# amathislab/HOISDF

Hardware: AMD Instinct MI355X
Metric: samples/sec (img + 2048 SDF queries) fwd+bwd at 1/2/4/8 MI355X (higher is better)
Workload: dtype f32 (emulated contractions, f32 accumulate, f16x2 form: operands as scaled hi + lo f16 pieces x 3 products - 22 operand bits, one power-of-two scale per ROW of a linear layer's row operand, per (sample, head) of the attention operands, per weight matrix; the attention backward's dS as three pieces x

## Files before the change

hoisdf_amd/_lib.py:

```python
from __future__ import annotations

import ctypes as C
import os
from typing import Dict, List

_HERE = os.path.dirname(os.path.abspath(__file__))
LIB_PATH = os.environ.get("HOISDF_LIB", os.path.join(_HERE, "libhoisdf_hip.so"))
HEADER_PATH = os.path.join(os.path.dirname(_HERE), "include", "hoisdf.h")
MAX_LEVELS = 8


class HoisdfLibraryError(RuntimeError):
    pass


class HoisdfError(RuntimeError):
    def __init__(self, code: int, msg: str):
        super().__init__(f"libhoisdf_hip status {code}: {msg}")
        self.code = code


class Pyramid(C.Structure):
    _fields_ = [("n_levels", C.c_int), ("B", C.c_int), ("data", C.c_void_p * MAX_LEVELS),
                ("C", C.c_int * MAX_LEVELS), ("H", C.c_int * MAX_LEVELS), ("W", C.c_int * MAX_LEVELS)]
# ... 157 lines not shown
    "hoisdf_attention_bwd": [_P, _I, _P, _I, _P, _I, _P, _I, _P, _I, _P, _P, _P, _P, _P, _I, _I, _I, _I,
                             _I, _F, _U64, _P],
    "hoisdf_attention_fwd_bf16x2": [_P, _I, _P, _I, _P, _I, _P, _I, _I, _I, _I, _I, _I, _P, _L, _P],
    "hoisdf_attention_fwd_emu": [_P, _I, _P, _I, _P, _I, _P, _I, _P, _I, _I, _I, _I, _I, _F, _U64, _P, _L, _I, _P],
    "hoisdf_attention_fwd_emu_mag": [_P, _I, _P, _I, _P, _I, _P, _I, _P, _I, _I, _I, _I, _I, _F, _U64, _P, _L, _I, _P, _P, _P, _P, _P],
    "hoisdf_attention_bwd_emu": [_P, _I, _P, _I, _P, _I, _P, _I, _P, _I, _P, _P, _P, _P, _P, _I, _I, _I, _I, _I, _F, _U64, _P, _P,
                                 _L, _P],
    "hoisdf_attention_bwd_emu_mag": [_P, _I, _P, _I, _P, _I, _P, _I, _P, _I, _P, _P, _P, _P, _P, _I, _I, _I, _I, _I, _F, _U64, _P, _P,
                                 _L, _P, _P, _P, _P, _P, _P],
    "hoisdf_attention_small_fwd": [_P, _I, _P, _I, _P, _I, _P, _P, _I, _P, _I, _I, _I, _I, _F, _U64, _P],
    "hoisdf_attention_small_bwd": [_P, _I, _P, _I, _P, _I, _P, _P, _I, _P, _P, _P, _I, _I, _I, _I, _F,
                                   _U64, _P],
    "hoisdf_add_layernorm_fwd": [_P, _P, _P, _P, _P, _P, _P, _L, _I, _F, _F, _U64, _P],
    "hoisdf_add_layernorm_bwd": [_P, _P, _P, _P, _P, _P, _P, _P, _P, _P, _P, _L, _I, _F, _U64, _P],
    "hoisdf_residual_dropout": [_P, _P, _P, _L, _I, _F, _U64, _P],
    "hoisdf_layernorm_rows_fwd": [_P, _P, _P, _P, _P, _P, _L, _I, _I, _I, _F, _P],
    "hoisdf_layernorm_rows_bwd": [_P, _P, _P, _P, _P, _P, _P, _P, _P, _L, _I, _I, _I, _P],
    "hoisdf_sdf_query_train_fwd": [_PYR, _P, _P, _L, _I, _P, _P, _F, _I, _I, _SDFW, _F, _F, _U64, _P, _P, _P, _P, _L, _P, _L, _P],
    "hoisdf_sdf_query_bwd": [_PYR, _P, _P, _L, _I, _P, _P, _F, _I, _I, _SDFW, _F, _F, _P, _L, _P, _P, _P, _L, _P],
    "hoisdf_sdf_infer_count": [_P, _P, _P, _F, _I, _I, _P, _P, _P, _P],
    "hoisdf_sdf_infer_count_begin": [_P, _P, _P, _F, _I, _I, _P, _P, _P],
    "hoisdf_sdf_infer": [_PYR, _P, _P, _P, _F, _I, _I, _P, _P, _I, _I, _I, _SDFW, _F, _F, _U64, _P, _P, _P, _P, _L, _P],
    "hoisdf_decoder_layer_fwd": [_P, _P, _P, _P, _P, _P, _P, _P, _P, _L, _P, _L, _P],
    "hoisdf_decoder_layer_bwd": [_P, _P, _P, _P, _P, _P, _P, _L, _P, _P, _P, _P, _I, _P, _P, _P, _L, _P],
    "hoisdf_encoder_layer_fwd": [_P, _P, _P, _P, _P, _P, _L, _P, _L, _P],
    "hoisdf_encoder_layer_bwd": [_P, _P, _P, _P, _P, _L, _P, _P, _P, _P, _P, _L, _P],
    "hoisdf_mano_prepare": [_P, _P, _P, _P, _P],
    "hoisdf_mano_head_fwd": [_P, _I, _I, _P, _I, _I, _P, _P, _P, _P, _P, _P, _P, _P, _P, _I, _I, _P, _P, _P, _P, _P],
    "hoisdf_mano_head_bwd": [_P, _P, _I, _P, _P, _P, _P, _P, _P, _P, _P, _P, _I, _I, _P, _P, _P, _P, _P, _P, _P],
    "hoisdf_vote_fwd": [_P, _P, _P, _P, _P, _I, _I, _I, _I, _P],
    "hoisdf_vote_bwd": [_P, _P, _P, _P, _P, _P, _P, _P, _I, _I, _I, _I, _P],
    "hoisdf_vote_loss_fwd": [_P, _P, _P, _P, _F, _P, _P, _P, _P, _P, _I, _I, _I, _I, _P],
    "hoisdf_vote_loss_bwd": [_P, _P, _P, _P, _F, _P, _P, _P, _P, _P, _P, _P, _I, _I, _I, _I, _P],
    "hoisdf_tokens_fwd": [_P, _P, _P, _P, _F, _I, _I, _P, _P, _P, _P, _P, _P, _P, _P, _P, _I, _I, _I, _I, _I, _P, _L, _P, _L, _P],
    "hoisdf_tokens_bwd": [_P, _P, _P, _P, _F, _I, _I, _P, _P, _P, _P, _P, _P, _L, _P, _P, _I, _P, _I, _I, _I, _I, _I, _P, _L, _P],
    "hoisdf_heads_vote_fwd": [_P, _P, _P, _P, _P, _F, _P, _P, _P, _P, _I, _I, _I, _I, _P, _L, _P, _L, _P],
    "hoisdf_heads_vote_bwd": [_P, _P, _P, _P, _P, _F, _P, _P, _L, _P, _P, _P, _P, _P, _P, _I, _I, _I, _I, _P, _L, _P],
    "hoisdf_point_loss_fwd": [_P, _P, _L, _L, _I, _L, _I, _F, _F, _F, _P, _P, _P],
    "hoisdf_point_loss_bwd": [_P, _P, _L, _L, _I, _L, _I, _F, _F, _F, _P, _P, _P],
    "hoisdf_pose_prepare": [_P, _P, _P, _L, _P],
    "hoisdf_pose_infer_begin": [_P, _P, _P, _P, _P, _P, _P, _P, _P],
    "hoisdf_pose_infer": [_P, _P, _PYR, _P, _P, _P, _P, _P, _P, _P, _P, _P, _L, _P, _P],
    "hoisdf_conv_pack_weight": [_P, _P, _P, _P, _P, _P, _F, _I, _I, _I, _I, _I, _P, _P, _P],
    "hoisdf_conv_plan": [_L, _I, _I, _I, _P, _P],
    "hoisdf_conv2d_fwd": [_P, _I, _P, _P, _P, _I, _P, _I, _I, _I, _I, _I, _I, _I, _I, _I, _I, _I, _I, _P, _L, _P],
    "hoisdf_conv_transpose2d_fwd": [_P, _I, _P, _P, _P, _I, _I, _I, _I, _I, _I, _I, _I, _P, _L, _P],
    "hoisdf_maxpool2d_fwd": [_P, _I, _P, _I, _I, _I, _I, _I, _P],
    "hoisdf_encoder_prepare": [_P, _P, _I, _P, _L, _P],
    "hoisdf_encoder_pyramid_shape": [_P, _PYR],
    "hoisdf_encoder_infer": [_P, _P, _P, _P, _P, _P, _L, _P],
}
_RET = {"hoisdf_version": C.c_char_p, "hoisdf_last_error": C.c_char_p}
_OTHER = {"hoisdf_set_deterministic": ([_I], None), "hoisdf_set_gemm_emu": ([_I], None), "hoisdf_get_gemm_emu": ([], C.c_int), "hoisdf_get_deterministic": ([], C.c_int),
          "hoisdf_mano_dirs_image_floats": ([], C.c_long),
          "hoisdf_point_loss_blocks": ([_L], C.c_int),
          "hoisdf_bn_workspace_floats": ([_L, _I], C.c_long),
          "hoisdf_token_build_bwd_partials": ([], C.c_int),
          "hoisdf_tokens_saved_bytes": ([_P, _L, _I], C.c_long),
          "hoisdf_tokens_workspace_bytes": ([_P, _L, _I], C.c_long),
          "hoisdf_heads_vote_saved_bytes": ([_P, _P, _I, _I, _I, _I], C.c_long),
          "hoisdf_heads_vote_workspace_bytes": ([_P, _P, _I, _I, _I, _I, _I], C.c_long),
          "hoisdf_sdf_infer_workspace": ([_L, _I, _I], C.c_long),
          "hoisdf_sdf_query_train_saved_bytes": ([_L, _I], C.c_long),
          "hoisdf_sdf_query_train_workspace_bytes": ([_L, _I, _I], C.c_long),
          "hoisdf_decoder_layer_saved_bytes": ([_P], C.c_long),
          "hoisdf_decoder_layer_workspace_bytes": ([_P, _I], C.c_long),
          "hoisdf_encoder_layer_saved_bytes": ([_P], C.c_long),
          "hoisdf_encoder_layer_out_mag": ([_P, _P], C.c_void_p),
          "hoisdf_encoder_layer_workspace_bytes": ([_P, _I], C.c_long),
          "hoisdf_sdf_query_workspace": ([_L, _I, _I], C.c_long),
          "hoisdf_linear_bwd_weight_workspace": ([_L, _I, _I], C.c_long),
          "hoisdf_linear_emu_image_bytes": ([_I, _I], C.c_long),
          "hoisdf_linear_emu_prepare_blocks": ([_I, _I, _I], C.c_long),
          "hoisdf_linear_bwd_weight_emu_workspace": ([_L, _I, _I], C.c_long),
          "hoisdf_linear_emu_supported": ([_P, _L, _I], C.c_int),
          "hoisdf_linear_emu_small_max_rows": ([], C.c_int),
          "hoisdf_linear_emu_pieces": ([], C.c_int),
          "hoisdf_mag_words": ([_L], C.c_long),
          "hoisdf_head_mag_words": ([_L, _I, _I], C.c_long),
          "hoisdf_linear_emu_small_supported": ([_P, _L, _P, _L, _L, _I, _I], C.c_int),
          "hoisdf_attention_bf16x2_workspace": ([_I, _I, _I, _I], C.c_long),
          "hoisdf_attention_emu_workspace": ([_I, _I, _I, _I, _I], C.c_long),
          "hoisdf_attention_bwd_emu_workspace": ([_I, _I, _I, _I, _I], C.c_long),
          "hoisdf_conv_packed_floats": ([_I, _I, _I, _I], C.c_long),
          "hoisdf_conv_workspace_bytes": ([_L, _I, _I, _I], C.c_long),
          "hoisdf_encoder_tensor_count": ([_P], C.c_int),
          "hoisdf_encoder_tensor_name": ([_P, _I], C.c_char_p),
          "hoisdf_encoder_tensor_numel": ([_P, _I], C.c_long),
          "hoisdf_encoder_prepared_bytes": ([_P], C.c_long),
          "hoisdf_encoder_infer_workspace": ([_P], C.c_long),
          "hoisdf_encoder_launch_count": ([_P], C.c_int),
          "hoisdf_pose_prepared_bytes": ([_P], C.c_long),
          "hoisdf_pose_infer_workspace": ([_P, _P], C.c_long)}

_lib = None


def lib() -> C.CDLL:
    global _lib
    if _lib is None:
        if not os.path.exists(LIB_PATH):
            raise HoisdfLibraryError(
                f"{LIB_PATH} not found: the HIP extension is not built (make -C hoisdf_amd/csrc). "
                "There is no CPU fallback for the hot path.")
        L = C.CDLL(LIB_PATH)
        for name, args in SIGNATURES.items():
# ... 38 lines not shown
```

hoisdf_amd/csrc/chain.h:

```cpp
#pragma once
#include <stdlib.h>

#include <mutex>
#include <unordered_map>

#include "common.h"

namespace hoisdf {
namespace {

constexpr long EMU_MIN_ROWS = 2048;
constexpr long EMU_DW_MIN_ROWS = 8192;

inline bool al16(const void* p) { return (reinterpret_cast<uintptr_t>(p) & 15) == 0; }

struct Bump {
  char* base; long cap; long off = 0; bool overflow = false;
  Bump(void* b, long c) : base(static_cast<char*>(b)), cap(c) {}
  void* take(long bytes) {
    off = (off + 255) & ~255L;
    const long at = off;
    off += bytes;
    if (!base) return nullptr;
    if (off > cap) { overflow = true; return nullptr; }
    return base + at;
  }
  float* floats(long n) { return static_cast<float*>(take(n * 4)); }
};

struct SavedMags {
  std::mutex mu;
  std::unordered_map<const void*, int> on;
  void put(const void* key, bool v) { if (!key) return; std::lock_guard<std::mutex> l(mu); if (on.size() > 8192) on.clear(); on[key] = v ? 1 : 0; }
  int get(const void* key) { std::lock_guard<std::mutex> l(mu); auto it = on.find(key); return it == on.end() ? -1 : it->second; }
};
inline SavedMags& saved_mags() { static SavedMags s; return s; }

struct Ctx {
  hipStream_t st; void* stream;
  Bump* ws;
  bool dry;
  bool emu;
  int rc = HOISDF_OK;
  bool ok() const { return rc == HOISDF_OK; }
};

inline bool emu_small(const Ctx& c, long M, const float* a, long lda, const float* W, long ldw, int N, int K) {
  if (!c.emu || M > hoisdf_linear_emu_small_max_rows() || N % 4 || K % 4 || lda % 4 || ldw % 4) return false;
  return c.dry || hoisdf_linear_emu_small_supported(a, lda, W, ldw, M, N, K);
}
bool emu_rows(const Ctx& c, long M, const float* a, long lda, int contraction) {
  return c.emu && M >= EMU_MIN_ROWS && contraction % 4 == 0 && lda % 4 == 0 && (c.dry || al16(a));
}
const void* image_of(Ctx& c, const void* given, const float* W, int ldw, int N, int K, int transpose) {
  if (given) return given;
  void* img = c.ws->take(hoisdf_linear_emu_image_bytes(transpose ? K : N, transpose ? N : K));
  if (c.dry) return nullptr;
  if (!img) { c.rc = HOISDF_ERR_WORKSPACE; return nullptr; }
  c.rc = hoisdf_linear_emu_prepare(W, ldw, N, K, transpose, img, c.stream);
  return img;
}
void lin_fwd(Ctx& c, const float* x, int ldx, const float* W, int ldw, const void* img, const float* b, float* y, int ldy, long M, int N,
             int K, int act, float p, uint64_t seed, uint32_t* bits, int K_pad = 0, const uint32_t* x_mag = nullptr, uint32_t* y_mag = nullptr,
             uint32_t* y_heads = nullptr, int head_L = 0) {
  if (!c.ok()) return;
  if (K_pad < K || (K_pad + 15) / 16 != (K + 15) / 16) K_pad = K;
  if (emu_rows(c, M, x, ldx, K_pad)) {
    const void* im = image_of(c, img, W, ldw, N, K, 0);
    if (c.dry || !c.ok()) return;
    c.rc = linear_fwd_emu_mag(x, ldx, im, b, y, ldy, M, N, K_pad, act, p, seed, bits, x_mag, y_mag, c.stream, y_heads, head_L);
    return;
  }
  if (c.dry) return;
  if (emu_small(c, M, x, ldx, W, ldw, N, K)) { c.rc = hoisdf_linear_fwd_emu_small(x, ldx, W, ldw, b, y, ldy, M, N, K, act, p, seed, bits, c.stream); return; }
  c.rc = hoisdf_linear_fwd(x, ldx, W, ldw, b, y, ldy, M, N, K, act, p, seed, bits, c.stream);
}
void lin_bwd_input(Ctx& c, const float* dy, int lddy, const uint32_t* bits, float p, const float* W, int ldw, const void* img_t, float* dx,
                   int lddx, long M, int N, int K, int accumulate, const uint32_t* dy_mag = nullptr, uint32_t* dx_mag = nullptr,
                   uint32_t* dx_heads = nullptr, int head_L = 0) {
  if (!c.ok()) return;
  if (!bits) p = 0.f;
  if (emu_rows(c, M, dy, lddy, N)) {
    const void* im = image_of(c, img_t, W, ldw, N, K, 1);
    if (c.dry || !c.ok()) return;
    c.rc = linear_bwd_input_emu_mag(dy, lddy, bits, p, im, dx, lddx, M, N, K, accumulate, dy_mag, accumulate ? nullptr : dx_mag, c.stream,
                                    accumulate ? nullptr : dx_heads, head_L);
    return;
  }
  if (c.dry) return;
  if (emu_small(c, M, dy, lddy, W, ldw, N, K)) { c.rc = hoisdf_linear_bwd_input_emu_small(dy, lddy, bits, p, W, ldw, dx, lddx, M, N, K, accumulate, c.stream); return; }
  c.rc = hoisdf_linear_bwd_input(dy, lddy, bits, p, W, ldw, dx, lddx, M, N, K, accumulate, c.stream);
}
void lin_bwd_weight(Ctx& c, const float* dy, int lddy, const uint32_t* bits, float p, const float* x, int ldx, float* dW, float* db, long M,
                    int N, int K, int K_pad = 0, const uint32_t* dy_mag = nullptr, const uint32_t* x_mag = nullptr) {
  if (!c.ok()) return;
  if (!bits) p = 0.f;
  if (K_pad < K) K_pad = K;
  const bool emu = c.emu && M >= EMU_DW_MIN_ROWS && (N < K ? N : K) >= 64 && N % 4 == 0 && K_pad % 4 == 0 && lddy % 4 == 0 && ldx % 4 == 0 &&
                   (c.dry || (al16(dy) && al16(x) && al16(dW)));
  if (emu) {
    const long nws = hoisdf_linear_bwd_weight_emu_workspace(M, N, K_pad);
    float* w = c.ws->floats(nws > 4 ? nws : 4);
    if (!c.dry) {
      if (!w) { c.rc = HOISDF_ERR_WORKSPACE; return; }
      if (dy_mag || x_mag) c.rc = linear_bwd_weight_emu_mag(dy, lddy, bits, p, x, ldx, dW, K_pad, db, M, N, K_pad, w, nws, dy_mag, x_mag, c.stream);
      else c.rc = hoisdf_linear_bwd_weight_emu(dy, lddy, bits, p, x, ldx, dW, K_pad, db, M, N, K_pad, w, nws, c.stream);
    }
    return;
  }
  if (c.emu && M <= hoisdf_linear_emu_small_max_rows()) {
    if (!c.dry) c.rc = hoisdf_linear_bwd_weight_emu_small(dy, lddy, bits, p, x, ldx, dW, K_pad, db, M, N, K_pad, c.stream);
    return;
  }
  long nws = 0; float* w = nullptr;
  if (deterministic_mode()) {
    nws = hoisdf_linear_bwd_weight_workspace(M, N, K_pad);
    if (nws > 0) w = c.ws->floats(nws);
    if (!c.dry && nws > 0 && !w) { c.rc = HOISDF_ERR_WORKSPACE; return; }
  }
  if (c.dry) return;
  c.rc = hoisdf_linear_bwd_weight(dy, lddy, bits, p, x, ldx, dW, K_pad, db, M, N, K_pad, w, nws, c.stream);
}


}
}
```

hoisdf_amd/csrc/common.h:

```cpp
#pragma once
#include <hip/hip_runtime.h>
#include <stdint.h>

#include "../../include/hoisdf.h"

namespace hoisdf {

void set_error(const char* fmt, ...);
int check_launch(const char* what);

#define HOISDF_REQUIRE(cond, code, ...)                 \
  do {                                                  \
    if (!(cond)) {                                      \
      ::hoisdf::set_error(__VA_ARGS__);                 \
      return (code);                                    \
    }                                                   \
  } while (0)

static inline hipStream_t as_stream(void* s) { return reinterpret_cast<hipStream_t>(s); }
static inline int cdiv(long a, long b) { return (int)((a + b - 1) / b); }

__device__ __forceinline__ uint32_t mix32(uint32_t x) {
  x ^= x >> 16; x *= 0x7feb352dU; x ^= x >> 15; x *= 0x846ca68bU; x ^= x >> 16;
  return x;
// ... 33 lines not shown
                          int H, int Lq, int Lk, int kv_len, float drop_p, uint64_t seed, void* workspace, long workspace_bytes, int keep,
                          uint32_t* o_mag, void* stream, const uint32_t* q_hm = nullptr, const uint32_t* k_hm = nullptr,
                          const uint32_t* v_hm = nullptr);
int attention_bwd_emu_mag(const float* q, int ldq, const float* k, int ldk, const float* v, int ldv, const float* o, int ldo,
                          const float* dout, int lddo, const float* lse, float* delta, float* dq, float* dk, float* dv, int B, int H,
                          int Lq, int Lk, int kv_len, float drop_p, uint64_t seed, const void* fwd_workspace, void* workspace,
                          long workspace_bytes, uint32_t* g_mag, void* stream, const uint32_t* q_hm = nullptr,
                          const uint32_t* k_hm = nullptr, const uint32_t* v_hm = nullptr, const uint32_t* do_hm = nullptr);

bool emu_form_h2();
int emu_rowmag_launch(const float* x, long ld, long M, int K, uint32_t* words, hipStream_t st);
int emu_mag_measure(const float* x, long ld, long M, int K, uint32_t* words, hipStream_t st);
int emu_headmag_launch(const float* x, long ld, long M, int groups, int L, uint32_t* words, hipStream_t st);
uint32_t* mag_scratch(hipStream_t st, long words);

__device__ __forceinline__ uint32_t mag_bits(float v) { return __builtin_bit_cast(uint32_t, v) & 0x7fffffffu; }
__device__ __forceinline__ uint32_t mag_bits4(const float4& v) {
  return max(max(mag_bits(v.x), mag_bits(v.y)), max(mag_bits(v.z), mag_bits(v.w)));
}
__device__ __forceinline__ void f16_saturate_on() { __builtin_amdgcn_s_setreg((0 << 11) | (23 << 6) | 1, 1); }
__device__ __forceinline__ void rowmag_publish_wave(uint32_t* words, long row, uint32_t m);
template <int CTRL>
__device__ __forceinline__ uint32_t dpp_u32(uint32_t v) { return (uint32_t)__builtin_amdgcn_update_dpp(0, (int)v, CTRL, 0xf, 0xf, true); }
template <int G>
__device__ __forceinline__ uint32_t group_max_u32(uint32_t m) {
  static_assert(G == 4 || G == 8 || G == 16 || G == 32 || G == 64, "group size");
  m = max(m, dpp_u32<0xB1>(m));
  m = max(m, dpp_u32<0x4E>(m));
  if (G >= 8) m = max(m, dpp_u32<0x141>(m));
  if (G >= 16) m = max(m, dpp_u32<0x140>(m));
  if (G >= 32) m = max(m, (uint32_t)__shfl_xor((int)m, 16, 64));
  if (G >= 64) m = max(m, (uint32_t)__shfl_xor((int)m, 32, 64));
  return m;
}
__device__ __forceinline__ void rowmag_publish_wave(uint32_t* words, long row, uint32_t m) {
  if (!words) return;
  m = group_max_u32<64>(m);
  if ((threadIdx.x & 63) == 0) atomicMax(words + row, m);
}
__device__ __forceinline__ uint32_t mag_exp(uint32_t amax_bits) { return min(max((amax_bits >> 23) & 0xffu, 14u), 254u); }
__device__ __forceinline__ float mag_scale(uint32_t amax_bits) { return __builtin_bit_cast(float, (267u - mag_exp(amax_bits)) << 23); }
__device__ __forceinline__ float mag_inv_scale(uint32_t amax_bits) { return __builtin_bit_cast(float, (mag_exp(amax_bits) - 13u) << 23); }
__device__ __forceinline__ uint32_t block_max_u32(uint32_t v, uint32_t* red4) {
#pragma unroll
  for (int o = 32; o >= 1; o >>= 1) v = max(v, (uint32_t)__shfl_xor((int)v, o));
  if ((threadIdx.x & 63) == 0) red4[threadIdx.x >> 6] = v;
  __syncthreads();
  return max(max(red4[0], red4[1]), max(red4[2], red4[3]));
}
__device__ __forceinline__ long head_words(long groups, long nb) { return groups * nb; }
int linear_fwd_emu_mag(const float* x, int ldx, const void* w_image, const float* bias, float* y, int ldy, long M, int N, int K, int act,
                       float drop_p, uint64_t seed, uint32_t* relu_bits, const uint32_t* x_mag, uint32_t* y_mag, void* stream,
                       uint32_t* y_heads = nullptr, int head_L = 0);
int linear_bwd_input_emu_mag(const float* dy, int lddy, const uint32_t* relu_bits, float drop_p, const void* wt_image, float* dx, int lddx,
                             long M, int N, int K, int accumulate, const uint32_t* dy_mag, uint32_t* dx_mag, void* stream,
                             uint32_t* dx_heads = nullptr, int head_L = 0);
int linear_bwd_weight_emu_mag(const float* dy, int lddy, const uint32_t* relu_bits, float drop_p, const float* x, int ldx, float* dW, int lddw,
                              float* db, long M, int N, int K, float* workspace, long workspace_floats, const uint32_t* dy_mag,
                              const uint32_t* x_mag, void* stream);
int project_gather_fwd_mag(const hoisdf_pyramid* pyr, const float* points, const int32_t* sample_idx, long n_rows, int rows_per_sample,
                           const float* center, const float* cam_intr, float scale, int img_h, int img_w, float* feat, int ldf, float* cam_out,
                           float* uv_out, uint32_t* feat_mag, void* stream);
int posenc_fwd_mag(const float* points, long n_rows, float* x0, int ldx0, int col0, float* pe, uint32_t* x0_mag, void* stream);
int sdf_head_bwd_mag(const float* dsdf, const float* sdf_raw, const float* h, int ldh, const float* w, float* dh, int lddh, float* dw,
                     float* db, long n_rows, int K, float clamp, uint32_t* dh_mag, void* stream);
int add_layernorm_fwd_mag(const float* x, const float* r, const float* gamma, const float* beta, float* y, float* mean, float* rstd, long M,
                          int D, float eps, float drop_p, uint64_t seed, uint32_t* y_mag, void* stream);
int add_layernorm_bwd_mag(const float* dy, const float* x, const float* r, const float* gamma, const float* mean, const float* rstd,
                          const float* dx_add, float* dx, float* dr, float* dgamma, float* dbeta, long M, int D, float drop_p, uint64_t seed,
                          uint32_t* dx_mag, uint32_t* dr_mag, void* stream);

struct ConvProblem {
  int B, H, W, C_in, C_out, KH, KW, stride, pad, act;
  int transposed;
};
struct ConvPlan {
  int tile;
  int splitk, k_per_split;
  long workspace_bytes;
};
ConvPlan conv_plan(long M, int N, int K, int ncls);
int conv_launch(const ConvProblem& c, const float* x, int ldx, const float* w_packed, const float* bias, const float* residual, int ldr,
                float* y, int ldy, int c_off, void* workspace, long workspace_bytes, hipStream_t st);
int conv_pack_launch(const float* w, const float* conv_bias, const float* gamma, const float* beta, const float* mean, const float* var,
                     float eps, int C_out, int C_in, int KH, int KW, int transposed, float* packed, float* bias_out, hipStream_t st);
int maxpool_launch(const float* x, int ldx, float* y, int ldy, int B, int H, int W, int C, hipStream_t st);

bool deterministic_mode();
bool gemm_emu_mode();
struct DetScratch {
  float* part;
  unsigned* ticket;
  int on;
};
DetScratch det_scratch(size_t floats);

__device__ __forceinline__ void block_column_sum(float* dstA, int nA, float* dstB, int nB,
                                                 const float* src, unsigned* s_last ,
                                                 const DetScratch ds) {
  const int n = nA + nB;
  if (!ds.on) {
    for (int c = threadIdx.x; c < n; c += blockDim.x) atomicAdd(c < nA ? dstA + c : dstB + (c - nA), src[c]);
    return;
  }
  for (int c = threadIdx.x; c < n; c += blockDim.x) ds.part[(size_t)blockIdx.x * n + c] = src[c];
  __threadfence();
  __syncthreads();
  if (threadIdx.x == 0) *s_last = (atomicAdd(ds.ticket, 1u) == gridDim.x - 1) ? 1u : 0u;
  __syncthreads();
  if (!*s_last) return;
  __threadfence();
  const volatile float* part = ds.part;
  for (int c = threadIdx.x; c < n; c += blockDim.x) {
    float acc = 0.f;
    for (unsigned b = 0; b < gridDim.x; ++b) acc += part[(size_t)b * n + c];
    if (c < nA) dstA[c] += acc; else dstB[c - nA] += acc;
  }
  if (threadIdx.x == 0) *ds.ticket = 0u;
}

#define SB() __builtin_amdgcn_sched_barrier(0)
#define PK_SUB(d, x, y) asm("v_pk_add_f32 %0, %1, %2 neg_lo:[0,1] neg_hi:[0,1]" : "=v"(d) : "v"(x), "v"(y))

__device__ __forceinline__ float wave_sum(float v) {
#pragma unroll
  for (int o = 32; o > 0; o >>= 1) v += __shfl_xor(v, o, 64);
  return v;
}
__device__ __forceinline__ float wave_max(float v) {
#pragma unroll
  for (int o = 32; o > 0; o >>= 1) v = fmaxf(v, __shfl_xor(v, o, 64));
  return v;
}

__device__ __forceinline__ int xcd_remap(int bid, int nblk) {
  const int nx = 8;
  int xcd = bid % nx, loc = bid / nx;
  int q = nblk / nx, r = nblk % nx;
  int base = xcd < r ? xcd * (q + 1) : r * (q + 1) + (xcd - r) * q;
  return base + loc;
}
// ... 3 lines not shown
```

hoisdf_amd/csrc/gemm_emu.h:

```cpp
#pragma once
#include "common.h"

namespace hoisdf {

typedef float f32x16 __attribute__((ext_vector_type(16)));
typedef float f32x4 __attribute__((ext_vector_type(4)));
typedef float f32x2 __attribute__((ext_vector_type(2)));
typedef __bf16 bf16x8 __attribute__((ext_vector_type(8)));
typedef __bf16 bf16x2 __attribute__((ext_vector_type(2)));
typedef _Float16 f16x8 __attribute__((ext_vector_type(8)));
typedef _Float16 f16x2 __attribute__((ext_vector_type(2)));
typedef unsigned int u32x4 __attribute__((ext_vector_type(4)));
typedef unsigned int u32x2 __attribute__((ext_vector_type(2)));
#define MFB(a, b, c) __builtin_amdgcn_mfma_f32_32x32x16_bf16((a), (b), (c), 0, 0, 0)
#define MFH(a, b, c) __builtin_amdgcn_mfma_f32_32x32x16_f16((a), (b), (c), 0, 0, 0)

constexpr int TM = 256, TN = 128, KS = 16, NT = 256;
constexpr int WN = TN / 2, NJ = WN / 32;
constexpr int A_U4 = 3 * 2 * TM, B_U4 = 3 * 2 * TN, STAGE_U4 = A_U4 + B_U4;
constexpr int NB = B_U4 / NT;
constexpr int HTM = 256, HTN = 256;
constexpr int HA_U4 = 2 * 2 * HTM, HB_U4 = 2 * 2 * HTN;
constexpr int H_TRAILER = 128;
constexpr int DT = 256;

#define SPLIT1(x, i)                             \
  do {                                           \
    const __bf16 a_ = (__bf16)(x);               \
    const float r1_ = (x) - (float)a_;           \
    const __bf16 b_ = (__bf16)r1_;               \
    const float r2_ = r1_ - (float)b_;           \
    p0[i] = a_; p1[i] = b_; p2[i] = (__bf16)r2_; \
  } while (0)
__device__ __forceinline__ void split3x8(const float4 u, const float4 w, bf16x8& p0, bf16x8& p1, bf16x8& p2) {
  SPLIT1(u.x, 0); SPLIT1(u.y, 1); SPLIT1(u.z, 2); SPLIT1(u.w, 3);
  SPLIT1(w.x, 4); SPLIT1(w.y, 5); SPLIT1(w.z, 6); SPLIT1(w.w, 7);
}

struct EmuArgs {
  const float* A; long lda;
  const u32x4* Bimg;
  float* C; int ldc;
  const float* bias;
  const uint32_t* abits; int ldbits; float ascale;
  uint32_t* bits_out; int ldbits_out;
  int M, N, K;
  int act; float drop_p, inv_keep; uint32_t thresh; uint64_t seed;
  int tiles_m, tiles_n, vecC, beta;
  QkvPlanes qkv;
  const uint32_t* a_amax; const float* b_scale;
  uint32_t* amax_out;
  uint32_t* head_out; int head_L, head_nb;
};

struct DwArgs {
  const float* dy; long lddy;
  const float* x; long ldx;
  const uint32_t* bits; int ldbits; float ascale;
  float* C; long c_split_stride;
  float* colsum; long colsum_split_stride;
  int M, N, K;
  int splitk, m_per_split, tiles_n, tiles_k;
  const uint32_t* dy_amax; const uint32_t* x_amax;
};

__device__ __forceinline__ uint32_t h2_exp(uint32_t amax_bits) { return mag_exp(amax_bits); }
__device__ __forceinline__ float h2_scale(uint32_t amax_bits) { return mag_scale(amax_bits); }
__device__ __forceinline__ float h2_inv_scale(uint32_t amax_bits) { return mag_inv_scale(amax_bits); }
__host__ __device__ __forceinline__ uint32_t* h2_trailer(void* image, int R, int Kc) {
  return reinterpret_cast<uint32_t*>(static_cast<char*>(image) + (size_t)((R + HTN - 1) / HTN) * ((Kc + KS - 1) / KS) * HB_U4 * 16);
}

#define EMU_PREP_FIND(items, n, lo)                                                                                    \
  int lo = 0, hi_ = (n) - 1;                                                                                           \
  while (lo < hi_) {                                                                                                   \
    const int mid_ = (lo + hi_ + 1) >> 1;                                                                              \
    if ((items)[mid_].first_block <= (long)blockIdx.x) lo = mid_; else hi_ = mid_ - 1;                                 \
  }

#define NOP_ ((void)0)
#define SYNC() do { SB(); __syncthreads(); SB(); } while (0)

#define EMU_A_DESCRIPTORS(TM_, arow0)                                                                                  \
  const int rows_in = min(TM_, g.M - m0);                                                                              \
  __amdgpu_buffer_rsrc_t rsa[4], rsm[4];                                                                               \
  _Pragma("unroll") for (int i = 0; i < 4; ++i) {                                                                      \
    const int rows_q = max(min(rows_in - i * 64, 64), 0);                              \
    rsa[i] = __builtin_amdgcn_make_buffer_rsrc(const_cast<float*>(g.A + ((size_t)(arow0) + i * 64) * g.lda), 0,        \
                                               rows_q > 0 ? (int)((((long)rows_q - 1) * g.lda + g.K) * 4) : 0, 0x00020000); \
    rsm[i] = __builtin_amdgcn_make_buffer_rsrc(const_cast<uint32_t*>(MASK ? g.abits + ((size_t)m0 + i * 64) * g.ldbits : nullptr), 0, \
                                               MASK ? (int)((long)rows_q * g.ldbits * 4) : 0, 0x00020000);             \
  }
#define EMU_A_SLOTS(TM_)                                                                                               \
  const int aoff = (int)((((long)wave * 16 + rl) * g.lda + 4 * qd) * 4);                                               \
  const int moff = (int)(((long)wave * 16 + rl) * g.ldbits * 4);                                                       \
  const int wslot = 2 * (cq * TM_ + ((wave * 16 + rl) ^ (cq << 2))) + (qd & 1);                                        \
  const int aread = (wm * 128 + l31) ^ (kh << 2);                                                                      \
  const int kq = g.K - 4 * qd;
#define EMU_LDGA(i, sl)                                                                                                \
  do {                                                                                                                 \
    const int k0_ = min((sl), last) * KS;                              \
    const f32x4 v_ = __builtin_bit_cast(f32x4, __builtin_amdgcn_raw_buffer_load_b128(rsa[i], aoff, k0_ * 4, 0));       \
    rp[2 * (i)] = f32x2{v_[0], v_[1]}; rp[2 * (i) + 1] = f32x2{v_[2], v_[3]};                                          \
    if (MASK) rm[i] = __builtin_amdgcn_raw_buffer_load_b32(rsm[i], moff, (k0_ >> 5) * 4, 0);                           \
  } while (0)
#define EMU_UI(i, sl) do { if (MASK) mb = rm[i] >> ((((sl) & 1) << 4) + 4 * qd); if (KTAIL) kin = (sl) * KS < kq; } while (0)
#define EMU_MASK_KTAIL(v_, p)                                                                                          \
  do {                                                                                                                 \
    if (MASK) {            \
      float xa_, xb_;      \
      asm("v_and_b32 %0, %1, %2" : "=v"(xa_) : "v"(__builtin_amdgcn_sbfe((int)mb, 2 * ((p) & 1), 1)), "v"(v_.x));       \
// ... 87 lines not shown
      const float sc = part == 0 ? g.qkv.qscale : 1.f;
      __bf16* const r0 = static_cast<__bf16*>(g.qkv.r[part][0]);
      __bf16* const r1 = static_cast<__bf16*>(g.qkv.r[part][1]);
      __bf16* const r2 = static_cast<__bf16*>(g.qkv.r[part][2]);
      const bool trn = part == 2 && g.qkv.vt[0] != nullptr;
#pragma unroll
      for (int i = 0; i < 4; ++i) {
#pragma unroll
        for (int j = 0; j < 2; ++j)
#pragma unroll
          for (int r = 0; r < 16; ++r) w[((r & 3) + 8 * (r >> 2) + 4 * kh) * ES + j * 32 + l31] = acc[i][2 * hh + j][r] * sc;
        if (r0) {
#pragma unroll
          for (int p = 0; p < 4; ++p) {
            const int rr = p * 8 + (lane >> 3), cc = (lane & 7) * 8;
            const float4 u = *reinterpret_cast<const float4*>(w + rr * ES + cc);
            const float4 v = *reinterpret_cast<const float4*>(w + rr * ES + cc + 4);
            bf16x8 p0, p1, p2;
            split3x8(u, v, p0, p1, p2);
            const size_t o = ((size_t)bh * g.qkv.Lp + s0 + i * 32 + rr) * 64 + cc;
            *reinterpret_cast<bf16x8*>(r0 + o) = p0;
            *reinterpret_cast<bf16x8*>(r1 + o) = p1;
            *reinterpret_cast<bf16x8*>(r2 + o) = p2;
          }
        }
        if (trn) {
          __bf16* const t0 = static_cast<__bf16*>(g.qkv.vt[0]);
          __bf16* const t1 = static_cast<__bf16*>(g.qkv.vt[1]);
          __bf16* const t2 = static_cast<__bf16*>(g.qkv.vt[2]);
#pragma unroll
          for (int q = 0; q < 4; ++q) {
            const float* c0 = w + (8 * q) * ES + lane;
            const float4 u = make_float4(c0[0], c0[ES], c0[2 * ES], c0[3 * ES]);
            const float4 v = make_float4(c0[4 * ES], c0[5 * ES], c0[6 * ES], c0[7 * ES]);
            bf16x8 p0, p1, p2;
            split3x8(u, v, p0, p1, p2);
            const size_t o = ((size_t)bh * 64 + lane) * g.qkv.Lp + s0 + i * 32 + 8 * q;
            *reinterpret_cast<bf16x8*>(t0 + o) = p0;
            *reinterpret_cast<bf16x8*>(t1 + o) = p1;
            *reinterpret_cast<bf16x8*>(t2 + o) = p2;
          }
        }
      }
    }
    return;
  }
  const bool full = (m0 + TM_ <= g.M) && (n0 + TN_ <= g.N);
  const bool stream_c = !g.beta && (long)g.M * g.N >= (16L << 20);
  if (full && g.vecC) {
    constexpr int ES = WN_ + 4, LPR = WN_ / 4, RPI = 64 / LPR;
    float* w = reinterpret_cast<float*>(lds) + wave * (32 * ES);
#pragma unroll
    for (int i = 0; i < 4; ++i) {
#pragma unroll
      for (int j = 0; j < NJ_; ++j)
#pragma unroll
        for (int r = 0; r < 16; ++r) w[((r & 3) + 8 * (r >> 2) + 4 * kh) * ES + j * 32 + l31] = acc[i][j][r];
      if (g.amax_out) {
        const float* rp = w + l31 * ES + kh * (WN_ / 2);
        float m = 0.f;
#pragma unroll
        for (int q = 0; q < WN_ / 8; ++q) {
          const float4 t = *reinterpret_cast<const float4*>(rp + 4 * q);
          m = __builtin_fmaxf(__builtin_fmaxf(m, __builtin_fabsf(t.x)), __builtin_fmaxf(__builtin_fabsf(t.y), __builtin_fmaxf(__builtin_fabsf(t.z), __builtin_fabsf(t.w))));
        }
        uint32_t mb = __builtin_bit_cast(uint32_t, m);
        mb = max(mb, (uint32_t)__shfl_xor((int)mb, 32, 64));
        if (kh == 0) atomicMax(g.amax_out + (m0 + wm * 128 + i * 32 + l31), mb);
      }
#pragma unroll
      for (int p = 0; p < 32 / RPI; ++p) {
        const int rr = p * RPI + lane / LPR, cc = (lane % LPR) * 4;
        float4 v = *reinterpret_cast<const float4*>(w + rr * ES + cc);
        float4* cp = reinterpret_cast<float4*>(g.C + (size_t)(m0 + wm * 128 + i * 32 + rr) * g.ldc + n0 + wn * WN_ + cc);
        if (g.beta) {
          const float4 old = *cp;
          v.x += old.x; v.y += old.y; v.z += old.z; v.w += old.w;
        }
        typedef float v4f_ __attribute__((ext_vector_type(4)));
#ifdef H2_ABL_NOSTORE
        if (g.seed != 0x5eed5eed5eedull) continue;
#endif
        if (stream_c) __builtin_nontemporal_store(v4f_{v.x, v.y, v.z, v.w}, reinterpret_cast<v4f_*>(cp));
        else *cp = v;
      }
    }
  } else {
#pragma unroll
    for (int j = 0; j < NJ_; ++j)
#pragma unroll
      for (int i = 0; i < 4; ++i)
#pragma unroll
        for (int r = 0; r < 16; ++r) {
          const int row = rbase + i * 32 + (r & 3) + 8 * (r >> 2), col = cbase + j * 32;
          if (row < g.M && col < g.N) {
            float* cp = g.C + (size_t)row * g.ldc + col;
            *cp = g.beta ? *cp + acc[i][j][r] : acc[i][j][r];
          }
        }
    if (g.amax_out) {
#pragma unroll
      for (int i = 0; i < 4; ++i)
#pragma unroll
        for (int r = 0; r < 16; ++r) {
          const int row = rbase + i * 32 + (r & 3) + 8 * (r >> 2);
          uint32_t mb = 0u;
#pragma unroll
          for (int j = 0; j < NJ_; ++j) if (cbase + j * 32 < g.N) mb = max(mb, mag_bits(acc[i][j][r]));
          mb = group_max_u32<32>(mb);
          if (l31 == 0 && row < g.M) atomicMax(g.amax_out + row, mb);
        }
    }
  }
  if (g.bits_out) {
    uint32_t wd[2][NJ_];
#pragma unroll
    for (int hh = 0; hh < 2; ++hh)
#pragma unroll
      for (int j = 0; j < NJ_; ++j) wd[hh][j] = 0u;
#pragma unroll
    for (int i = 0; i < 4; ++i)
#pragma unroll
      for (int r = 0; r < 16; ++r) {
        const int rl = (i & 1) * 32 + (r & 3) + 8 * (r >> 2);
#pragma unroll
        for (int j = 0; j < NJ_; ++j) {
          const unsigned long long q = __ballot(acc[i][j][r] > 0.f);
          if (lane == rl) wd[i >> 1][j] = (uint32_t)q;
          if (lane == rl + 4) wd[i >> 1][j] = (uint32_t)(q >> 32);
        }
      }
    const int wcol = (n0 + wn * WN_) >> 5;
    const int nvalid = g.N - (n0 + wn * WN_);
#pragma unroll
    for (int hh = 0; hh < 2; ++hh) {
      const int row = m0 + wm * 128 + hh * 64 + lane;
      if (row < g.M) {
#pragma unroll
        for (int j = 0; j < NJ_; ++j) {
          const int nv = nvalid - 32 * j;
          if (nv > 0) g.bits_out[(size_t)row * g.ldbits_out + wcol + j] = nv >= 32 ? wd[hh][j] : (wd[hh][j] & ((1u << nv) - 1u));
        }
      }
    }
  }
}

int emu_b3_prepare(const float* W, int ldw, int R, int Kc, int transpose, void* image, hipStream_t st);
int emu_b3_prepare_batch(const hoisdf_emu_prep_item* d_items, int n, long total_blocks, hipStream_t st);
int emu_b3_launch(EmuArgs g, hipStream_t st);
// ... 8 lines not shown
```

hoisdf_amd/csrc/gemm_emu.hip:

```cpp
#include <stdlib.h>

#include <map>
#include <mutex>
#include <unordered_map>
#include <utility>

#include "gemm_emu.h"

namespace hoisdf {

__global__ __launch_bounds__(256) void emu_rowmag_kernel(const float* __restrict__ x, long ld, long M, int K, uint32_t* __restrict__ words) {
  constexpr int RPW = 8;
  const int lane = threadIdx.x & 63;
  const long row0 = ((long)blockIdx.x * 4 + (threadIdx.x >> 6)) * RPW;
  const int k4 = K >> 2;
  uint32_t m[RPW];
#pragma unroll
  for (int r = 0; r < RPW; ++r) {
    m[r] = 0u;
    if (row0 + r < M)
      for (int c = lane; c < k4; c += 64) {
        const u32x4 v = *reinterpret_cast<const u32x4*>(x + (row0 + r) * ld + 4 * c);
        m[r] = max(m[r], max(max(v[0] & 0x7fffffffu, v[1] & 0x7fffffffu), max(v[2] & 0x7fffffffu, v[3] & 0x7fffffffu)));
      }
// ... 168 lines not shown
  HOISDF_REQUIRE(hoisdf_linear_emu_supported(x, ldx, K), HOISDF_ERR_INVALID,
                 "linear_fwd_emu: x must be 16-byte aligned with ldx and K multiples of 4 (use hoisdf_linear_fwd otherwise)");
  EmuArgs g{};
  g.A = x; g.lda = ldx; g.Bimg = static_cast<const u32x4*>(w_image);
  g.C = y; g.ldc = ldy; g.bias = bias; g.M = (int)M; g.N = N; g.K = K;
  g.act = act; g.drop_p = drop_p; g.inv_keep = 1.f / (1.f - drop_p); g.thresh = drop_threshold(drop_p); g.seed = seed;
  g.bits_out = relu_bits; g.ldbits_out = (N + 31) / 32;
  g.a_amax = x_mag; g.amax_out = y_mag;
  if (y_heads) {
    HOISDF_REQUIRE(head_L > 0 && N % 64 == 0, HOISDF_ERR_INVALID, "linear_fwd_emu: head magnitudes need N %% 64 == 0 and the rows per sample");
    g.head_out = y_heads; g.head_L = head_L; g.head_nb = cdiv(M, head_L);
  }
  return launch_emu(g, as_stream(stream));
}

int hoisdf::linear_fwd_emu_qkv(const float* x, int ldx, const void* w_image, const float* bias, long M, int N, int K,
                               const QkvPlanes& pl, void* stream, const uint32_t* x_mag) {
  HOISDF_REQUIRE(x && w_image && M > 0 && N > 0 && K > 0 && ldx >= K && M < (1L << 31), HOISDF_ERR_INVALID, "linear_fwd_emu_qkv: bad arguments");
  HOISDF_REQUIRE(hoisdf_linear_emu_supported(x, ldx, K), HOISDF_ERR_INVALID, "linear_fwd_emu_qkv: x alignment / K");
  HOISDF_REQUIRE(pl.on && pl.L > 0 && pl.L % 128 == 0 && M % pl.L == 0 && N % 64 == 0 && pl.E % 64 == 0 && pl.Lp >= pl.L &&
                     pl.col0 % 64 == 0 && pl.col0 + N <= 3 * pl.E,
                 HOISDF_ERR_INVALID, "linear_fwd_emu_qkv: plane geometry (L=%d Lp=%d N=%d E=%d col0=%d)", pl.L, pl.Lp, N, pl.E, pl.col0);
  EmuArgs g{};
  g.A = x; g.lda = ldx; g.Bimg = static_cast<const u32x4*>(w_image);
  g.C = nullptr; g.ldc = N; g.bias = bias; g.M = (int)M; g.N = N; g.K = K;
  g.inv_keep = 1.f; g.qkv = pl;
  g.a_amax = x_mag;
  return launch_emu(g, as_stream(stream));
}

extern "C" int hoisdf_linear_fwd_emu_heads(const float* x, int ldx, const void* w_image, const float* bias, float* y, int ldy, long M, int N,
                                           int K, const uint32_t* x_mag, uint32_t* y_mag, uint32_t* y_heads, int L, void* stream) {
  HOISDF_REQUIRE(y_heads, HOISDF_ERR_INVALID, "linear_fwd_emu_heads: y_heads is required");
  return linear_fwd_emu_mag(x, ldx, w_image, bias, y, ldy, M, N, K, 0, 0.f, 0, nullptr, x_mag, y_mag, stream, y_heads, L);
}
extern "C" int hoisdf_linear_bwd_input_emu_heads(const float* dy, int lddy, const void* wt_image, float* dx, int lddx, long M, int N, int K,
                                                 const uint32_t* dy_mag, uint32_t* dx_mag, uint32_t* dx_heads, int L, void* stream) {
  HOISDF_REQUIRE(dx_heads, HOISDF_ERR_INVALID, "linear_bwd_input_emu_heads: dx_heads is required");
  return linear_bwd_input_emu_mag(dy, lddy, nullptr, 0.f, wt_image, dx, lddx, M, N, K, 0, dy_mag, dx_mag, stream, dx_heads, L);
}
extern "C" int hoisdf_linear_bwd_input_emu(const float* dy, int lddy, const uint32_t* relu_bits, float drop_p,
                                           const void* wt_image, float* dx, int lddx, long M, int N, int K, int accumulate,
                                           void* stream) {
  return linear_bwd_input_emu_mag(dy, lddy, relu_bits, drop_p, wt_image, dx, lddx, M, N, K, accumulate, nullptr, nullptr, stream);
}
extern "C" int hoisdf_linear_bwd_input_emu_mag(const float* dy, int lddy, const uint32_t* relu_bits, float drop_p,
                                               const void* wt_image, float* dx, int lddx, long M, int N, int K, int accumulate,
                                               const uint32_t* dy_mag, uint32_t* dx_mag, void* stream) {
  return linear_bwd_input_emu_mag(dy, lddy, relu_bits, drop_p, wt_image, dx, lddx, M, N, K, accumulate, dy_mag, dx_mag, stream);
}

int hoisdf::linear_bwd_input_emu_mag(const float* dy, int lddy, const uint32_t* relu_bits, float drop_p, const void* wt_image, float* dx,
                                     int lddx, long M, int N, int K, int accumulate, const uint32_t* dy_mag, uint32_t* dx_mag,
                                     void* stream, uint32_t* dx_heads, int head_L) {
  HOISDF_REQUIRE(M == 0 || (dy && wt_image && dx), HOISDF_ERR_INVALID, "linear_bwd_input_emu: null pointer");
  HOISDF_REQUIRE(M >= 0 && N > 0 && K > 0 && lddy >= N && lddx >= K && M < (1L << 31) && drop_p >= 0.f && drop_p < 1.f,
                 HOISDF_ERR_INVALID, "linear_bwd_input_emu: bad sizes");
  if (M == 0) return HOISDF_OK;
  HOISDF_REQUIRE(hoisdf_linear_emu_supported(dy, lddy, N), HOISDF_ERR_INVALID,
                 "linear_bwd_input_emu: dy must be 16-byte aligned with lddy and N multiples of 4");
  EmuArgs g{};
  g.A = dy; g.lda = lddy; g.Bimg = static_cast<const u32x4*>(wt_image);
  g.abits = relu_bits; g.ldbits = (N + 31) / 32; g.ascale = 1.f / (1.f - drop_p);
  g.C = dx; g.ldc = lddx; g.M = (int)M; g.N = K; g.K = N;
  g.inv_keep = 1.f;
  g.beta = accumulate ? 1 : 0;
  g.a_amax = dy_mag; g.amax_out = dx_mag;
  if (dx_heads) {
    HOISDF_REQUIRE(head_L > 0 && K % 64 == 0 && !accumulate, HOISDF_ERR_INVALID, "linear_bwd_input_emu: head magnitudes need K %% 64 == 0, the rows per sample, no accumulation");
    g.head_out = dx_heads; g.head_L = head_L; g.head_nb = cdiv(M, head_L);
  }
  return launch_emu(g, as_stream(stream));
}

extern "C" long hoisdf_linear_bwd_weight_emu_workspace(long M, int N, int K) {
  if (M <= 0 || N <= 0 || K <= 0) return 0;
  int splitk, mper;
  plan_dw(M, N, K, splitk, mper);
  if (splitk <= 1) return 0;
  return (long)splitk * ((long)N * K + N);
}

namespace {
int bwd_weight_emu(const float* dy, int lddy, const uint32_t* relu_bits, float drop_p, const float* x, int ldx, float* dW, int lddw,
                   float* db, long M, int N, int K, float* workspace, long workspace_floats, bool h2, const uint32_t* dy_mag,
                   const uint32_t* x_mag, void* stream) {
  HOISDF_REQUIRE(dW && (M == 0 || (dy && x)), HOISDF_ERR_INVALID, "linear_bwd_weight_emu: null pointer");
  HOISDF_REQUIRE(M > 0 && N > 0 && K > 0 && lddy >= N && ldx >= K && lddw == K && M < (1L << 31) && drop_p >= 0.f && drop_p < 1.f,
                 HOISDF_ERR_INVALID, "linear_bwd_weight_emu: bad sizes (a dense dW, lddw == K, is required)");
  HOISDF_REQUIRE(al16(dy) && al16(x) && al16(dW) && (lddy % 4 == 0) && (ldx % 4 == 0) && (N % 4 == 0) && (K % 4 == 0),
                 HOISDF_ERR_INVALID, "linear_bwd_weight_emu: operands must be 16-byte aligned with N, K and leading dims multiples of 4");
  hipStream_t st = as_stream(stream);
  DwArgs g{};
  g.dy = dy; g.lddy = lddy; g.x = x; g.ldx = ldx;
  g.bits = relu_bits; g.ldbits = (N + 31) / 32; g.ascale = 1.f / (1.f - drop_p);
  g.M = (int)M; g.N = N; g.K = K;
  const int dtk = dw_tile(K);
  g.tiles_n = cdiv(N, DT); g.tiles_k = cdiv(K, dtk);
  plan_dw(M, N, K, g.splitk, g.m_per_split);
  const long need = g.splitk > 1 ? (long)g.splitk * ((long)N * K + N) : 0;
  HOISDF_REQUIRE(need == 0 || (workspace && workspace_floats >= need && al16(workspace)), HOISDF_ERR_WORKSPACE,
                 "linear_bwd_weight_emu: workspace of %ld floats needed", need);
  if (g.splitk > 1) {
    g.C = workspace; g.c_split_stride = (long)N * K;
    g.colsum = db ? workspace + (size_t)g.splitk * N * K : nullptr; g.colsum_split_stride = N;
  } else {
    g.C = dW; g.c_split_stride = 0; g.colsum = db; g.colsum_split_stride = 0;
  }
  if (dtk == 256 && h2) {
    g.dy_amax = dy_mag; g.x_amax = x_mag;
    if (!dy_mag) {
      uint32_t* part = mag_scratch(st, M);
      if (!part) { set_error("linear_bwd_weight_emu: cannot allocate the row magnitudes"); return HOISDF_ERR_LAUNCH; }
      mag_trace("grad-weight dy", M, N);
      if (int rc = emu_rowmag_launch(dy, lddy, M, N, part, st)) return rc;
      g.dy_amax = part;
    }
    if (!x_mag) {
      uint32_t* part = mag_scratch(st, M);
      if (!part) { set_error("linear_bwd_weight_emu: cannot allocate the row magnitudes"); return HOISDF_ERR_LAUNCH; }
      mag_trace("grad-weight x", M, K);
      if (int rc = emu_rowmag_launch(x, ldx, M, K, part, st)) return rc;
      g.x_amax = part;
    }
  }
  return emu_dw_launch(g, h2, dW, db, workspace, st);
}
}

extern "C" int hoisdf_linear_bwd_weight_emu(const float* dy, int lddy, const uint32_t* relu_bits, float drop_p, const float* x,
                                            int ldx, float* dW, int lddw, float* db, long M, int N, int K, float* workspace,
                                            long workspace_floats, void* stream) {
  return bwd_weight_emu(dy, lddy, relu_bits, drop_p, x, ldx, dW, lddw, db, M, N, K, workspace, workspace_floats, false, nullptr, nullptr, stream);
}
int hoisdf::linear_bwd_weight_emu_mag(const float* dy, int lddy, const uint32_t* relu_bits, float drop_p, const float* x, int ldx,
                                      float* dW, int lddw, float* db, long M, int N, int K, float* workspace, long workspace_floats,
                                      const uint32_t* dy_mag, const uint32_t* x_mag, void* stream) {
  return bwd_weight_emu(dy, lddy, relu_bits, drop_p, x, ldx, dW, lddw, db, M, N, K, workspace, workspace_floats, form_h2(), dy_mag, x_mag, stream);
}
extern "C" int hoisdf_linear_bwd_weight_emu_mag(const float* dy, int lddy, const uint32_t* relu_bits, float drop_p, const float* x,
                                                int ldx, float* dW, int lddw, float* db, long M, int N, int K, float* workspace,
                                                long workspace_floats, const uint32_t* dy_mag, const uint32_t* x_mag, void* stream) {
  return linear_bwd_weight_emu_mag(dy, lddy, relu_bits, drop_p, x, ldx, dW, lddw, db, M, N, K, workspace, workspace_floats, dy_mag, x_mag, stream);
}
```

hoisdf_amd/csrc/gemm_emu_b3.hip:

```cpp
#include "gemm_emu.h"

namespace hoisdf {

__device__ __forceinline__ void emu_prep_weight_unit(const float* __restrict__ W, int ldw, int R, int Kc, int transpose, int nslab,
                                                     long idx, u32x4* __restrict__ img) {
  const int r = (int)(idx % TN);
  const int c = (int)((idx / TN) % 2);
  const int s = (int)((idx / (2 * TN)) % nslab);
  const int tn = (int)(idx / ((long)2 * TN * nslab));
  const int row = tn * TN + r;
  const int k0 = s * KS + c * 8;
  float e[8];
#pragma unroll
  for (int i = 0; i < 8; ++i) {
    const int k = k0 + i;
    float v = 0.f;
    if (row < R && k < Kc) v = transpose ? W[(size_t)k * ldw + row] : W[(size_t)row * ldw + k];
    e[i] = v;
  }
  bf16x8 p0, p1, p2;
  split3x8(make_float4(e[0], e[1], e[2], e[3]), make_float4(e[4], e[5], e[6], e[7]), p0, p1, p2);
  const size_t base = ((size_t)(tn * nslab + s) * 3) * 2 * TN;
  img[base + (0 * 2 + c) * TN + r] = __builtin_bit_cast(u32x4, p0);
  img[base + (1 * 2 + c) * TN + r] = __builtin_bit_cast(u32x4, p1);
// ... 84 lines not shown
      STA(st, i, t0, 0); STA(st, i, t1, 1); STA(st, i, t2, 2);                                                         \
    }                                                                                                                  \
    _Pragma("unroll") for (int q = 0; q < NB; ++q) STB(st, q);                                                         \
  } while (0)
#define LOAD_ALL(sl)                                                                                                   \
  do {                                                                                                                 \
     \
     \
    SB(); LDGA(0, sl); SB();                                                                                           \
    _Pragma("unroll") for (int q = 0; q < NB; ++q) { LDGB(q, sl); SB(); }                                              \
    _Pragma("unroll") for (int i = 1; i < 4; ++i) { LDGA(i, sl); SB(); }                                               \
  } while (0)
  LOAD_ALL(0);
  STAGE_ALL(st0, 0);
  LOAD_ALL(1);
  __syncthreads();
#pragma unroll
  for (int i = 0; i < 4; ++i) { aQ[i] = LDA(st0, 2, i); aP[i] = LDA(st0, 1, i); }
#pragma unroll
  for (int j = 0; j < NJ; ++j) { bP[j] = LDB(st0, 0, j); b1[j] = LDB(st0, 1, j); b2[j] = LDB(st0, 2, j); }
  MM(aQ, bP);
#pragma unroll
  for (int i = 0; i < 4; ++i) aQ[i] = LDA(st0, 0, i);
  MM(aP, b1); MM(aP, bP);
  STAGE_ALL(st1, 1);
  LOAD_ALL(2);
  SYNC();
  for (int s = 1; s + 1 < nslab2; s += 2) {
    PHASE(st1, st0, s, aQ, aP, bP, bQ);
    SYNC();
    PHASE(st0, st1, s + 1, aP, aQ, bQ, bP);
    SYNC();
  }
  PHASE(st1, st0, nslab2 - 1, aQ, aP, bP, bQ);
  SB();
  MM(aP, b2); MM(aP, b1); MM(aP, bQ);
  __syncthreads();
#undef LDGA
#undef LDGB
#undef UI
#undef U1
#undef U2
#undef U3
#undef U4
#undef STA
#undef STB
#undef LDA
#undef LDB
#undef M1
#undef MM
#undef PHASE
#undef STAGE_ALL
#undef LOAD_ALL
  emu_epilogue<TM, TN, NJ>(g, acc, st0, m0, n0, wm, wn, wave, lane, l31, kh, MASK ? g.ascale : 1.f);
}

int emu_b3_prepare(const float* W, int ldw, int R, int Kc, int transpose, void* image, hipStream_t st) {
  const int nslab = cdiv(Kc, KS);
  const long total = (long)cdiv(R, TN) * nslab * 2 * TN;
  hipLaunchKernelGGL(emu_prep_weight_kernel, dim3((unsigned)((total + 255) / 256)), dim3(256), 0, st, W, ldw, R, Kc, transpose, nslab, total,
                     static_cast<u32x4*>(image));
  return check_launch("linear_emu_prepare");
}

int emu_b3_prepare_batch(const hoisdf_emu_prep_item* d_items, int n, long total_blocks, hipStream_t st) {
  hipLaunchKernelGGL(emu_prep_weight_batch_kernel, dim3((unsigned)total_blocks), dim3(256), 0, st, d_items, n);
  return check_launch("linear_emu_prepare_batch");
}

int emu_b3_launch(EmuArgs g, hipStream_t st) {
  g.tiles_m = cdiv(g.M, TM);
  g.tiles_n = cdiv(g.N, TN);
  const bool kt = g.K % KS != 0 || (cdiv(g.K, KS) & 1);
  static void (*const kernel[2][2])(EmuArgs) = {{emu_kc2_kernel<false, false>, emu_kc2_kernel<false, true>},
                                                {emu_kc2_kernel<true, false>, emu_kc2_kernel<true, true>}};
  hipLaunchKernelGGL(kernel[g.abits != nullptr][kt], dim3((unsigned)(g.tiles_m * g.tiles_n)), dim3(NT), 0, st, g);
  return check_launch("linear_emu");
}

}
```

hoisdf_amd/csrc/gemm_emu_dw.hip:

```cpp
#include "gemm_emu.h"

namespace hoisdf {

namespace {
__device__ __forceinline__ uint64_t uni64(uint64_t v) {
  const uint32_t lo = __builtin_amdgcn_readfirstlane((uint32_t)v), hi = __builtin_amdgcn_readfirstlane((uint32_t)(v >> 32));
  return ((uint64_t)hi << 32) | lo;
}
}

#define DW_TILE_SETUP(DTK_)                                                                                            \
  const int tid = threadIdx.x, lane = tid & 63, wave = tid >> 6;                                                       \
  const int wm = wave >> 1, wn = wave & 1;                                                                             \
  const int l31 = lane & 31, kh = lane >> 5;                                                                           \
  const int ntile = g.tiles_n * g.tiles_k;                                                                             \
  const int bid = blockIdx.x;                                                                                          \
  const int split = (bid & 7) + 8 * (bid / (8 * ntile));       \
  const int t = (bid >> 3) % ntile;                                                                                    \
  if (split >= g.splitk) return;                                                                                       \
  const int tn = t / g.tiles_k, tk = t - tn * g.tiles_k;                                                               \
  const int n0 = tn * DT, k0 = tk * DTK_;                                                                              \
  const int mbeg = split * g.m_per_split;                                                                              \
  const int mend = min(g.M, mbeg + g.m_per_split);                                                                     \
  const int nslab = (mend - mbeg + KS - 1) / KS;
// ... 275 lines not shown
#define DU4(j, pr) do { f32x2 w_; PK_SUB(w_, rp_, fu_); t2[pr] = __builtin_bit_cast(uint32_t, __builtin_convertvector(w_, bf16x2)); } while (0)
#define DSTA(st, j, pl) (st)[wbase + ((j) ^ sw) + (pl) * 2 * DT] = ((pl) == 0 ? u32x4{t0[0], t0[1], t0[2], t0[3]} : (pl) == 1 ? u32x4{t1[0], t1[1], t1[2], t1[3]} : u32x4{t2[0], t2[1], t2[2], t2[3]})
#define DLA(st, p, i) __builtin_bit_cast(bf16x8, (st)[aread + ((p) * 2 + kh) * DT + (i) * 32])
#define DLB(st, p, j) __builtin_bit_cast(bf16x8, (st)[bread + ((p) * 2 + kh) * DT + (j) * 32])
#define M1(ax, bx, i, j, work) do { acc[i][j] = MFB(ax[i], bx[j], acc[i][j]); work; SB(); } while (0)
#define MM(ax, bx) _Pragma("unroll") for (int i = 0; i < 4; ++i) _Pragma("unroll") for (int j = 0; j < 4; ++j) acc[i][j] = MFB(ax[i], bx[j], acc[i][j])
#include "dw2_phase.inc"
#define DSTAGE_ALL(st)                                                                                                 \
  do {                                                                                                                 \
    _Pragma("unroll") for (int j = 0; j < 4; ++j) {                                                                    \
      _Pragma("unroll") for (int pr = 0; pr < 4; ++pr) { DU1(j, pr); DU2(j, pr); DU3(j, pr); DU4(j, pr); }             \
      DSTA(st, j, 0); DSTA(st, j, 1); DSTA(st, j, 2);                                                                  \
    }                                                                                                                  \
  } while (0)

  const int nslab2 = (max(nslab, 1) + 1) & ~1;
  bf16x8 aX[4], aY[4], aZ[4], bP[4], bQ[4], bR[4];
  DLOAD_ALL(0);
  DLOADM_ALL(0);
  DSTAGE_ALL(s0);
  DLOAD_ALL(1);
  DLOADM_ALL(1);
  __syncthreads();
#pragma unroll
  for (int i = 0; i < 4; ++i) { aZ[i] = DLA(s0, 0, i); aX[i] = DLA(s0, 1, i); aY[i] = DLA(s0, 2, i); }
#pragma unroll
  for (int j = 0; j < 4; ++j) { bQ[j] = DLB(s0, 0, j); bP[j] = DLB(s0, 1, j); bR[j] = DLB(s0, 2, j); }
  MM(aZ, bR); MM(aZ, bP); MM(aZ, bQ);
  DSTAGE_ALL(s1);
  DLOAD_ALL(2);
  DLOADM_ALL(2);
  SYNC();
  for (int s = 1; s + 1 < nslab2; s += 2) {
    DPHASE(s1, s0, s, aX, aY, aZ, bP, bQ, bR);
    SYNC();
    DPHASE(s0, s1, s + 1, aX, aY, aZ, bR, bQ, bP);
    SYNC();
  }
  DPHASE(s1, s0, nslab2 - 1, aX, aY, aZ, bP, bQ, bR);
  SB();
  MM(aX, bR); MM(aX, bQ); MM(aY, bQ);
  __syncthreads();
#undef DU1
#undef DU2
#undef DU3
#undef DU4
#undef DSTA
#undef DLA
#undef DLB
#undef M1
#undef MM
#undef DPHASE
#undef DSTAGE_ALL
  const float post = MASK ? g.ascale : 1.f;
  u32x4* lds = s0;
  DW2_STORE_COLSUM();
  DW_EPILOGUE(DT, MASK ? acc[i][j][r] * post : acc[i][j][r]);
}

template <bool MASK, bool HASDB>
__global__ __launch_bounds__(NT, 1) void emu_dw2h_kernel(DwArgs g) {
  constexpr int A_U4 = 2 * 2 * DT;
  constexpr int STG = 2 * A_U4;
  constexpr int EPI = (4 * 32 * (DT / 2 + 4) * 4 + 15) / 16;
  __shared__ __attribute__((aligned(16))) u32x4 lds_all[2 * STG > EPI ? 2 * STG : EPI];
  __shared__ uint32_t red4[4];
  u32x4* const s0 = lds_all;
  u32x4* const s1 = lds_all + STG;
  DW_TILE_SETUP(DT)
  f16_saturate_on();
  uint32_t am_dy = 0u, am_x = 0u;
  for (int i = mbeg + (int)threadIdx.x; i < mend; i += NT) { am_dy = max(am_dy, g.dy_amax[i]); am_x = max(am_x, g.x_amax[i]); }
  am_dy = block_max_u32(am_dy, red4);
  __syncthreads();
  am_x = block_max_u32(am_x, red4);

  f32x16 acc[4][4];
#pragma unroll
  for (int i = 0; i < 4; ++i)
#pragma unroll
    for (int j = 0; j < 4; ++j)
#pragma unroll
      for (int r = 0; r < 16; ++r) acc[i][j][r] = 0.f;

  DW2_STAGING_SETUP(A_U4)
  uint32_t t0[4], t1[4];
  const float sc = isA ? h2_scale(am_dy) : h2_scale(am_x);
  f32x2 rp_, fu_;
  f32x4 csum = {0.f, 0.f, 0.f, 0.f};
#define DU1(j, pr)                                                                                                     \
  do {                                                                                                                 \
    f32x2 v_ = (j) < 2 ? f32x2{rvL[2 * (pr)][(j) & 1], rvL[2 * (pr) + 1][(j) & 1]} : f32x2{rvH[2 * (pr)][(j) & 1], rvH[2 * (pr) + 1][(j) & 1]}; \
    if (MASK) {                                                                                                        \
      if ((j) == 0) {                                                                                                  \
        const uint32_t n0_ = ((rm[2 * (pr)] | notA) >> bsh) & 0xfu, n1_ = ((rm[2 * (pr) + 1] | notA) >> bsh) & 0xfu;   \
        mpk = ((pr) == 0 ? 0u : mpk) | (n0_ << (8 * (pr))) | (n1_ << (8 * (pr) + 4));                                  \
      }                                                                                                                \
      float xa_, xb_;                                                              \
      asm("v_and_b32 %0, %1, %2" : "=v"(xa_) : "v"(__builtin_amdgcn_sbfe((int)mpk, 8 * (pr) + (j), 1)), "v"(v_.x));    \
      asm("v_and_b32 %0, %1, %2" : "=v"(xb_) : "v"(__builtin_amdgcn_sbfe((int)mpk, 8 * (pr) + 4 + (j), 1)), "v"(v_.y)); \
      v_ = f32x2{xa_, xb_};                                                                                            \
    }                                                                                                                  \
    if (HASDB) csum[j] += v_.x + v_.y;                                                                                 \
    v_ *= sc;                                                                                                          \
    const f16x2 h_ = __builtin_convertvector(v_, f16x2);                       \
    t0[pr] = __builtin_bit_cast(uint32_t, h_); rp_ = v_;                                                               \
    fu_ = __builtin_convertvector(h_, f32x2);                                                                          \
  } while (0)
#define DU2(j, pr) do { f32x2 w_; PK_SUB(w_, rp_, fu_); t1[pr] = __builtin_bit_cast(uint32_t, __builtin_convertvector(w_, f16x2)); } while (0)
#define DSTA(st, j, pl) (st)[wbase + ((j) ^ sw) + (pl) * 2 * DT] = ((pl) == 0 ? u32x4{t0[0], t0[1], t0[2], t0[3]} : u32x4{t1[0], t1[1], t1[2], t1[3]})
#define DLA(st, p, i) __builtin_bit_cast(f16x8, (st)[aread + ((p) * 2 + kh) * DT + (i) * 32])
#define DLB(st, p, j) __builtin_bit_cast(f16x8, (st)[bread + ((p) * 2 + kh) * DT + (j) * 32])
#define M1(ax, bx, i, j, work) do { acc[i][j] = MFH(ax[i], bx[j], acc[i][j]); work; SB(); } while (0)
#define MM(ax, bx) _Pragma("unroll") for (int i = 0; i < 4; ++i) _Pragma("unroll") for (int j = 0; j < 4; ++j) acc[i][j] = MFH(ax[i], bx[j], acc[i][j])
#include "dw2h_phase.inc"
#define DSTAGE_ALL(st)                                                                                                 \
  do {                                                                                                                 \
    _Pragma("unroll") for (int j = 0; j < 4; ++j) {                                                                    \
      _Pragma("unroll") for (int pr = 0; pr < 4; ++pr) { DU1(j, pr); DU2(j, pr); }                                     \
      DSTA(st, j, 0); DSTA(st, j, 1);                                                                                  \
    }                                                                                                                  \
  } while (0)

  const int nslab2 = (max(nslab, 1) + 1) & ~1;
  f16x8 aH[4], aL[4], bP[4], bQ[4], bL[4];
  DLOAD_ALL(0);
  DLOADM_ALL(0);
  DSTAGE_ALL(s0);
  DLOAD_ALL(1);
  DLOADM_ALL(1);
  __syncthreads();
#pragma unroll
  for (int i = 0; i < 4; ++i) { aL[i] = DLA(s0, 1, i); aH[i] = DLA(s0, 0, i); }
#pragma unroll
  for (int j = 0; j < 4; ++j) { bP[j] = DLB(s0, 0, j); bL[j] = DLB(s0, 1, j); }
  MM(aL, bP); MM(aH, bL);
  DSTAGE_ALL(s1);
  DLOAD_ALL(2);
  DLOADM_ALL(2);
  SYNC();
  for (int s = 1; s + 1 < nslab2; s += 2) {
    DHPHASE(s1, s0, s, bP, bQ);
    SYNC();
    DHPHASE(s0, s1, s + 1, bQ, bP);
    SYNC();
  }
  DHPHASE(s1, s0, nslab2 - 1, bP, bQ);
  SB();
  MM(aH, bQ);
  __syncthreads();
#undef DU1
#undef DU2
#undef DSTA
#undef DLA
#undef DLB
#undef M1
#undef MM
#undef DHPHASE
#undef DSTAGE_ALL
  const float unscale = h2_inv_scale(am_dy) * h2_inv_scale(am_x);
  const float post = MASK ? g.ascale : 1.f;
  u32x4* lds = lds_all;
  DW2_STORE_COLSUM();
  DW_EPILOGUE(DT, acc[i][j][r] * (MASK ? post * unscale : unscale));
}

__global__ __launch_bounds__(1024) void emu_reduce_partials_kernel(const float* __restrict__ part, long stride, int splits,
                                                                   float* __restrict__ out, long n, int blocks0,
                                                                   const float* __restrict__ part1, long stride1,
                                                                   float* __restrict__ out1, long n1) {
  __shared__ float4 red[16][64];
  const int lane = threadIdx.x & 63, w = threadIdx.x >> 6;
  int blk = blockIdx.x;
  if (blk >= blocks0) { blk -= blocks0; part = part1; stride = stride1; out = out1; n = n1; }
  const long i = ((long)blk * 64 + lane) * 4;
  float4 s = make_float4(0.f, 0.f, 0.f, 0.f);
  if (i < n) {
    const float* p = part + i;
    int k = w;
    for (; k + 16 < splits; k += 32) {
      const float4 u = *reinterpret_cast<const float4*>(p + (size_t)k * stride);
      const float4 v = *reinterpret_cast<const float4*>(p + (size_t)(k + 16) * stride);
      s.x += u.x; s.y += u.y; s.z += u.z; s.w += u.w;
      s.x += v.x; s.y += v.y; s.z += v.z; s.w += v.w;
    }
    if (k < splits) {
      const float4 u = *reinterpret_cast<const float4*>(p + (size_t)k * stride);
      s.x += u.x; s.y += u.y; s.z += u.z; s.w += u.w;
    }
  }
  red[w][lane] = s;
  __syncthreads();
  if (w == 0 && i < n) {
    float4 t = red[0][lane];
#pragma unroll
    for (int j = 1; j < 16; ++j) {
      const float4 v = red[j][lane];
      t.x += v.x; t.y += v.y; t.z += v.z; t.w += v.w;
    }
    *reinterpret_cast<float4*>(out + i) = t;
  }
}

int dw_tile(int K) { return K <= 128 ? 128 : 256; }
void plan_dw(long M, int N, int K, int& splitk, int& mper) {
  const int dtk = dw_tile(K);
  const int ntile = cdiv(N, DT) * cdiv(K, dtk);
  const int slabs = cdiv(M, KS);
  const int slots = dtk == 256 ? 256 : 512;
  const int per_xcd = slots / 8 / ntile;
  int want = per_xcd >= 1 ? per_xcd * 8 : (ntile >= slots ? 1 : slots / ntile);
  if (want > slabs / 8) want = slabs / 8 > 0 ? slabs / 8 : 1;
  mper = cdiv(slabs, want) * KS;
  splitk = cdiv(M, mper);
}

int emu_dw_launch(const DwArgs& g, bool h2, float* dW, float* db, float* workspace, hipStream_t st) {
// ... 33 lines not shown
```

hoisdf_amd/csrc/gemm_emu_h2.hip:

```cpp
#include "gemm_emu.h"

namespace hoisdf {

__device__ __forceinline__ void h2_weight_amax_unit(const float* __restrict__ W, int ldw, int N, int K, int part, uint32_t* trailer, uint32_t* red4) {
  uint32_t m = 0u;
  const long n = (long)N * K;
  for (long i = (long)part * 256 + threadIdx.x; i < n; i += 16 * 256) {
    const long r = i / K;
    m = max(m, __builtin_bit_cast(uint32_t, W[r * ldw + (i - r * K)]) & 0x7fffffffu);
  }
  m = block_max_u32(m, red4);
  if (threadIdx.x == 0) trailer[part] = m;
}
__device__ __forceinline__ void h2_prep_weight_unit(const float* __restrict__ W, int ldw, int R, int Kc, int transpose, int nslab,
                                                    long idx, u32x4* __restrict__ img) {
  uint32_t* tr = h2_trailer(img, R, Kc);
  uint32_t am = 0u;
#pragma unroll
  for (int i = 0; i < 16; ++i) am = max(am, tr[i]);
  const float sc = h2_scale(am);
  if (idx == 0) {
    reinterpret_cast<float*>(tr)[16] = sc; reinterpret_cast<float*>(tr)[17] = h2_inv_scale(am);
#pragma unroll
    for (int i = 18; i < H_TRAILER / 4; ++i) tr[i] = 0u;
// ... 89 lines not shown
  const __amdgpu_buffer_rsrc_t rsb = __builtin_amdgcn_make_buffer_rsrc(
      const_cast<u32x4*>(g.Bimg + (size_t)tb * nslab * HB_U4), 0, nslab * HB_U4 * 16, 0x00020000);
  const int boff = NJ == 4 ? tid * 16 : ((tid >> 7) * HTN + r0 + (tid & 127)) * 16;
  EMU_A_SLOTS(HTM)
  f32x2 rp[8], fu[8];
  uint32_t t0[8], t1[8];
  u32x4 rb[NJ];
  uint32_t rm[4] = {0xffffffffu, 0xffffffffu, 0xffffffffu, 0xffffffffu}, mb = 0xfu;
  bool kin = true;
#define HLDGA(i, sl) EMU_LDGA(i, sl)
#define HLDGB(q, sl) rb[q] = __builtin_amdgcn_raw_buffer_load_b128(rsb, boff + (q) * ((NJ == 4 ? NT : 2 * HTN) * 16), min((sl), last) * (HB_U4 * 16), 0)
#define HUI(i, sl) EMU_UI(i, sl)
#define HC1(p)                                                                                                         \
  do {                                                                                                                 \
    f32x2 v_ = rp[p];                                                                                                  \
    EMU_MASK_KTAIL(v_, p);                                                                                             \
    v_ *= sAr[(p) >> 1];                                                                                               \
    const f16x2 h_ = __builtin_convertvector(v_, f16x2);                                                               \
    t0[p] = __builtin_bit_cast(uint32_t, h_); rp[p] = v_;                                                              \
    fu[p] = __builtin_convertvector(h_, f32x2);                                                                        \
  } while (0)
#define HC2(p) do { f32x2 w_; PK_SUB(w_, rp[p], fu[p]); t1[p] = __builtin_bit_cast(uint32_t, __builtin_convertvector(w_, f16x2)); } while (0)
#define HSTA(st, i, tp, pl) reinterpret_cast<u32x2*>(st)[wslot + (i) * 128 + (pl) * 4 * HTM] = u32x2{tp[2 * (i)], tp[2 * (i) + 1]}
#define HSTB(st, q) (st)[HA_U4 + tid + (q) * NT] = rb[q]
#define HLA(st, p, i) __builtin_bit_cast(f16x8, (st)[aread + ((p) * 2 + kh) * HTM + (i) * 32])
#define HLB(st, p, j) __builtin_bit_cast(f16x8, (st)[HA_U4 + wn * (TN_ / 2) + l31 + ((p) * 2 + kh) * TN_ + (j) * 32])
#define HM1(ax, bx, i, j, work) do { acc[i][j] = MFH(ax[i], bx[j], acc[i][j]); work; SB(); } while (0)
#define HMM(ax, bx) _Pragma("unroll") for (int i = 0; i < 4; ++i) _Pragma("unroll") for (int j = 0; j < NJ; ++j) acc[i][j] = MFH(ax[i], bx[j], acc[i][j])
#include "h2_phase.inc"
#define HSTAGE_ALL(st, sl)                                                                                             \
  do {                                                                                                                 \
    _Pragma("unroll") for (int i = 0; i < 4; ++i) {                                                                    \
      HUI(i, sl);                                                                                                      \
      HC1(2 * i); HC2(2 * i); HC1(2 * i + 1); HC2(2 * i + 1);                                                          \
      HSTA(st, i, t0, 0); HSTA(st, i, t1, 1);                                                                          \
    }                                                                                                                  \
    _Pragma("unroll") for (int q = 0; q < NJ; ++q) HSTB(st, q);                                                        \
  } while (0)
#define HLOAD_ALL(sl)                                                                                                  \
  do {                                                                                                                 \
     \
    SB();                                                                                                              \
    _Pragma("unroll") for (int q = 0; q < NJ; ++q) { HLDGB(q, sl); SB(); }                                             \
    _Pragma("unroll") for (int i = 0; i < 4; ++i) { HLDGA(i, sl); SB(); }                                              \
  } while (0)

  const int nslab2 = (nslab + 1) & ~1;
  f16x8 aH[4], aL[4], bP[NJ], bQ[NJ], bL[NJ];
  HLOAD_ALL(0);
#pragma unroll
  for (int i = 0; i < 4; ++i) sAr[i] = h2_scale(wrow[i]);
  HSTAGE_ALL(st0, 0);
  HLOAD_ALL(1);
  rpost[tid] = h2_inv_scale(wpost) * g.b_scale[1] * (MASK ? g.ascale : 1.f);
  __syncthreads();
#pragma unroll
  for (int i = 0; i < 4; ++i) { aL[i] = HLA(st0, 1, i); aH[i] = HLA(st0, 0, i); }
#pragma unroll
  for (int j = 0; j < NJ; ++j) { bP[j] = HLB(st0, 0, j); bL[j] = HLB(st0, 1, j); }
  HMM(aL, bP); HMM(aH, bL);
  HSTAGE_ALL(st1, 1);
  HLOAD_ALL(2);
  SYNC();
#define HPH(cur, nxt, s, bC, bN) do { if constexpr (NJ == 4) { HPHASE(cur, nxt, s, bC, bN); } else { HPHASE2(cur, nxt, s, bC, bN); } } while (0)
  for (int s = 1; s + 1 < nslab2; s += 2) {
    HPH(st1, st0, s, bP, bQ);
    SYNC();
    HPH(st0, st1, s + 1, bQ, bP);
    SYNC();
  }
  HPH(st1, st0, nslab2 - 1, bP, bQ);
  SB();
  HMM(aH, bQ);
  __syncthreads();
#undef HLDGA
#undef HLDGB
#undef HUI
#undef HC1
#undef HC2
#undef HSTA
#undef HSTB
#undef HLA
#undef HLB
#undef HM1
#undef HMM
#undef HPHASE
#undef HPHASE2
#undef HPH
#undef HSTAGE_ALL
#undef HLOAD_ALL
  emu_epilogue<HTM, TN_, NJ>(g, acc, st0, m0, n0, wm, wn, wave, lane, l31, kh, 1.f, rpost);
}

int emu_h2_prepare(const float* W, int ldw, int N, int K, int transpose, void* image, hipStream_t st) {
  const int R = transpose ? K : N, Kc = transpose ? N : K;
  const int nslab = cdiv(Kc, KS);
  const long total = (long)cdiv(R, HTN) * nslab * 2 * HTN;
  hipLaunchKernelGGL(h2_weight_amax_kernel, dim3(16), dim3(256), 0, st, W, ldw, N, K, R, Kc, image);
  hipLaunchKernelGGL(h2_prep_weight_kernel, dim3((unsigned)((total + 255) / 256)), dim3(256), 0, st, W, ldw, R, Kc, transpose, nslab, total,
                     static_cast<u32x4*>(image));
  return check_launch("linear_emu_prepare (f16x2)");
}

int emu_h2_prepare_batch(const hoisdf_emu_prep_item* d_items, int n, long total_blocks, hipStream_t st) {
  hipLaunchKernelGGL(h2_weight_amax_batch_kernel, dim3((unsigned)n * 16), dim3(256), 0, st, d_items);
  hipLaunchKernelGGL(h2_prep_weight_batch_kernel, dim3((unsigned)total_blocks), dim3(256), 0, st, d_items, n);
  return check_launch("linear_emu_prepare_batch (f16x2)");
// ... 18 lines not shown
```

hoisdf_amd/csrc/heads.hip:

```cpp
#include "chain.h"

using namespace hoisdf;

namespace {
constexpr int MLP_MAX = HOISDF_MLP_MAX_LAYERS;
inline long bits_words(int N) { return (N + 31) / 32; }

struct MlpSaved { float* h[MLP_MAX]; uint32_t* bits[MLP_MAX]; uint32_t* mag; };

bool mlp_ok(const hoisdf_mlp* m) {
  if (!m || m->n_layers < 1 || m->n_layers > MLP_MAX) return false;
  for (int i = 0; i <= m->n_layers; ++i) if (m->dims[i] <= 0) return false;
  return true;
}
void mlp_carve(const hoisdf_mlp* m, long M, Bump& b, MlpSaved& s) {
  const int last = m->n_layers - 1;
  for (int i = 0; i < m->n_layers; ++i) {
    s.h[i] = i < last ? b.floats(M * m->dims[i + 1]) : nullptr;
    const bool act = i < last || m->act_last;
    s.bits[i] = act ? static_cast<uint32_t*>(b.take(M * bits_words(m->dims[i + 1]) * 4)) : nullptr;
  }
  s.mag = static_cast<uint32_t*>(b.take((long)m->n_layers * M * 4));
}
inline bool chain_mags_on(const Ctx& c, long M) { return c.emu && emu_form_h2() && M >= EMU_MIN_ROWS; }
uint32_t* chain_mags(Ctx& c, long M, int n) {
  if (!chain_mags_on(c, M)) return nullptr;
  uint32_t* p = static_cast<uint32_t*>(c.ws->take((long)n * M * 4));
  if (c.dry || !p || !c.ok()) return nullptr;
  if (hipMemsetAsync(p, 0, (size_t)n * M * 4, c.st) != hipSuccess) { c.rc = HOISDF_ERR_LAUNCH; return nullptr; }
  return p;
}
void mlp_forward(Ctx& c, const hoisdf_mlp* m, const float* x, int ldx, long M, const MlpSaved& s, float* y, int ldy, const uint32_t* x_mag = nullptr) {
  const int last = m->n_layers - 1;
  const float* in = x; int ldin = ldx;
  uint32_t* mg = chain_mags_on(c, M) && !c.dry && s.mag && c.ok() ? s.mag : nullptr;
  if (!c.dry) saved_mags().put(s.mag, mg != nullptr);
  if (mg && hipMemsetAsync(mg, 0, (size_t)m->n_layers * M * 4, c.st) != hipSuccess) { c.rc = HOISDF_ERR_LAUNCH; return; }
  const uint32_t* in_mag = mg ? x_mag : nullptr;
  if (mg && !in_mag && emu_rows(c, M, x, ldx, m->dims[0])) {
    if ((c.rc = emu_mag_measure(x, ldx, M, m->dims[0], mg, c.st)) != HOISDF_OK) return;
    in_mag = mg;
  }
  for (int i = 0; i < m->n_layers; ++i) {
    float* out = i < last ? s.h[i] : y;
    const int ldo = i < last ? m->dims[i + 1] : ldy;
    uint32_t* out_mag = mg && i < last && emu_rows(c, M, in, ldin, m->dims[i]) ? mg + (long)(i + 1) * M : nullptr;
    lin_fwd(c, in, ldin, m->w[i], m->dims[i], m->img[i], m->b[i], out, ldo, M, m->dims[i + 1], m->dims[i], s.bits[i] ? 1 : 0, 0.f, 0, s.bits[i], 0,
            in_mag, out_mag);
    in = out; ldin = ldo; in_mag = out_mag;
  }
}
void mlp_backward(Ctx& c, const hoisdf_mlp* m, const hoisdf_mlp_grads* G, const float* x, int ldx, long M, const MlpSaved& s, const float* dy,
                  int lddy, float* dx, int lddx, int accumulate_dx, const uint32_t* x_mag = nullptr) {
  const float* g = dy; int ldg = lddy;
  const int last = m->n_layers - 1;
  uint32_t* mg = chain_mags(c, M, m->n_layers + 1);
  const bool fwd_mags = mg && s.mag && saved_mags().get(s.mag) != 0;
  const uint32_t* g_mag = nullptr;
  if (mg && emu_rows(c, M, dy, lddy, m->dims[last + 1])) {
    if ((c.rc = emu_mag_measure(dy, lddy, M, m->dims[last + 1], mg + (long)(last + 1) * M, c.st)) != HOISDF_OK) return;
    g_mag = mg + (long)(last + 1) * M;
  }
  for (int i = last; i >= 0; --i) {
    const float* in = i > 0 ? s.h[i - 1] : x;
    const int ldin = i > 0 ? m->dims[i] : ldx;
    const uint32_t* in_mag = !fwd_mags ? nullptr : i > 0 ? (emu_rows(c, M, i > 1 ? s.h[i - 2] : x, i > 1 ? m->dims[i - 1] : ldx, m->dims[i - 1]) ? s.mag + (long)i * M : nullptr)
                                                         : (x_mag ? x_mag : (emu_rows(c, M, x, ldx, m->dims[0]) ? s.mag : nullptr));
    lin_bwd_weight(c, g, ldg, s.bits[i], 0.f, in, ldin, G->dw[i], G->db[i], M, m->dims[i + 1], m->dims[i], 0, g_mag, g_mag ? in_mag : nullptr);
    if (i == 0 && !dx) break;
    float* gin = i > 0 ? c.ws->floats(M * m->dims[i]) : dx;
    const int ldgin = i > 0 ? m->dims[i] : lddx;
    if (!c.dry && c.ok() && !gin) { c.rc = HOISDF_ERR_WORKSPACE; return; }
    uint32_t* gin_mag = mg && i > 0 && emu_rows(c, M, g, ldg, m->dims[i + 1]) ? mg + (long)i * M : nullptr;
    lin_bwd_input(c, g, ldg, s.bits[i], 0.f, m->w[i], m->dims[i], m->img_t[i], gin, ldgin, M, m->dims[i + 1], m->dims[i], i == 0 ? accumulate_dx : 0,
                  g_mag, gin_mag);
    g = gin; ldg = ldgin; g_mag = gin_mag;
  }
}
const uint32_t* enc_mag(const Ctx& c, const hoisdf_mlp* m, const float* x, int ldx, long M, const MlpSaved& s) {
  return chain_mags_on(c, M) && !c.dry && s.mag && saved_mags().get(s.mag) != 0 && emu_rows(c, M, x, ldx, m->dims[0]) ? s.mag : nullptr;
}
bool grads_ok(const hoisdf_mlp* m, const hoisdf_mlp_grads* G) {
  if (!G) return false;
  for (int i = 0; i < m->n_layers; ++i) if (!G->dw[i] || !G->db[i]) return false;
  return true;
}

struct TokSaved { float* feat; float* fea; MlpSaved mlp; };
void tok_carve(const hoisdf_mlp* m, long M, bool own_feat, Bump& b, TokSaved& s) {
  s.feat = own_feat ? b.floats(M * m->dims[0]) : nullptr;
  s.fea = b.floats(M * m->dims[m->n_layers]);
  mlp_carve(m, M, b, s.mlp);
}

struct VoteSaved { float *off, *cls, *stats; MlpSaved vote, cl; };
void vote_carve(const hoisdf_mlp* mv, const hoisdf_mlp* mc, long M, int LB, int J, Bump& b, VoteSaved& s) {
  s.off = b.floats(M * 3 * J); s.cls = b.floats(M * J); s.stats = b.floats((long)LB * J * 2);
  mlp_carve(mv, M, b, s.vote); mlp_carve(mc, M, b, s.cl);
}
}

extern "C" long hoisdf_tokens_saved_bytes(const hoisdf_mlp* mlp, long n_rows, int gather_inside) {
  if (!mlp_ok(mlp) || n_rows <= 0) return 0;
  Bump b(nullptr, 0); TokSaved s;
  tok_carve(mlp, n_rows, gather_inside != 0, b, s);
  return b.off + 256;
}

static int tokens_backward(const hoisdf_mlp* mlp, const hoisdf_mlp_grads* G, const float* feat, long M, TokSaved& s, const float* dtok,
                           const float* sdf, const float* beta, float* dfeat, int accumulate_dfeat, float* dbeta, int B, int P, int S, int row0,
                           int D, Bump& ws, bool dry, void* stream) {
  Ctx c{as_stream(stream), stream, &ws, dry, gemm_emu_mode()};
  const int F = mlp->dims[mlp->n_layers];
  float* dfea = ws.floats(M * F);
  float* part = ws.floats(hoisdf_token_build_bwd_partials());
  if (!dry) {
    if (!dfea || !part) { set_error("tokens_bwd: workspace too small"); return HOISDF_ERR_WORKSPACE; }
    c.rc = hoisdf_token_build_bwd_ordered(dtok, s.fea, F, sdf, beta, dfea, F, dbeta, part, B, P, S, row0, D, stream);
  }
  mlp_backward(c, mlp, G, feat, mlp->dims[0], M, s.mlp, dfea, F, dfeat, mlp->dims[0], accumulate_dfeat);
  if (c.ok() && !dry && ws.overflow) { set_error("tokens_bwd: workspace too small"); return HOISDF_ERR_WORKSPACE; }
  return c.rc;
}

extern "C" long hoisdf_tokens_workspace_bytes(const hoisdf_mlp* mlp, long n_rows, int backward_pass) {
  if (!mlp_ok(mlp) || n_rows <= 0) return 0;
  Bump ws(nullptr, 0), sv(nullptr, 0);
  TokSaved s; tok_carve(mlp, n_rows, false, sv, s);
  Ctx c{nullptr, nullptr, &ws, true, gemm_emu_mode()};
// ... 145 lines not shown
```

hoisdf_amd/csrc/layers.hip:

```cpp
#include <stdlib.h>

#include <mutex>
#include <unordered_map>

#include "chain.h"

namespace hoisdf {
namespace {

__global__ void rows_copy_add_kernel(float* __restrict__ dst, long dst_gs, const float* __restrict__ src, long src_gs, int rows, int E4,
                                     long total, int add) {
  const long i = (long)blockIdx.x * blockDim.x + threadIdx.x;
  if (i >= total) return;
  const long per = (long)rows * E4;
  const long g = i / per, r = i - g * per;
  float4* d = reinterpret_cast<float4*>(dst + g * dst_gs) + r;
  const float4 s = reinterpret_cast<const float4*>(src + g * src_gs)[r];
  if (add) { float4 t = *d; t.x += s.x; t.y += s.y; t.z += s.z; t.w += s.w; *d = t; }
  else *d = s;
}
int rows_copy_add(float* dst, long dst_gs, const float* src, long src_gs, int groups, int rows, int E, int add, hipStream_t st) {
  const long total = (long)groups * rows * (E / 4);
  if (total == 0) return HOISDF_OK;
  hipLaunchKernelGGL(rows_copy_add_kernel, dim3((unsigned)cdiv(total, 256)), dim3(256), 0, st, dst, dst_gs, src, src_gs, rows, E / 4, total, add);
// ... 138 lines not shown
  } else if (!dry && c.ok()) {
    c.rc = hoisdf_attention_fwd(q, ldq, k, ldkv, v, ldkv, s.o, E, s.lse, g.B, g.H, g.nq, g.S, g.S, g.p, d->seed[0], stream);
  }
  lin_fwd(c, s.o, E, w->w_out, E, w->img_out, w->b_out, s.a, E, g.M, E, E, 0, 0.f, 0, nullptr, 0, o_mag, nullptr);
  float* st = s.st;
  if (!dry && c.ok()) c.rc = add_layernorm_fwd_mag(xq2, s.a, w->g1, w->be1, s.x1, st, st + g.M, g.M, E, g.eps, g.p, d->seed[1], mg(MAG_X1), stream);
  lin_fwd(c, s.x1, E, w->w1, E, w->img_1, w->b1, s.h, F, g.M, F, E, 1, g.p, d->seed[2], s.bits, 0, mg(MAG_X1), mg(MAG_H));
  lin_fwd(c, s.h, F, w->w2, F, w->img_2, w->b2, s.f, E, g.M, E, F, 0, 0.f, 0, nullptr, 0, mg(MAG_H), nullptr);
  if (!dry && c.ok()) c.rc = add_layernorm_fwd_mag(s.x1, s.f, w->g2, w->be2, x_out, st + 2 * g.M, st + 3 * g.M, g.M, E, g.eps, g.p, d->seed[3], mg(MAG_XOUT), stream);
  if (w->g3 && !dry && c.ok()) {
    if (g.ni == g.nq) c.rc = hoisdf_add_layernorm_fwd(x_out, nullptr, w->g3, w->be3, y_out, st + 4 * g.M, st + 5 * g.M, g.M, E, g.eps, 0.f, 0, stream);
    else c.rc = hoisdf_layernorm_rows_fwd(x_out, w->g3, w->be3, y_out, st + 4 * g.M, st + 5 * g.M, g.B, g.nq, g.ni, E, g.eps, stream);
  }
  if (c.ok() && !dry && (ws.overflow || saved.overflow)) { set_error("encoder_layer_fwd: workspace / saved buffer too small"); return HOISDF_ERR_WORKSPACE; }
  return c.rc;
}

int backward(const float* x, const float* x_out, const hoisdf_encoder_layer_weights* w, const hoisdf_encoder_layer_desc* d, const Geo& g,
             Bump& saved, const float* g_x_out, const float* g_y, float* dx, const hoisdf_encoder_layer_grads* G, Bump& ws, bool dry,
             void* stream, bool fwd_mags = true) {
  Ctx c{as_stream(stream), stream, &ws, dry, gemm_emu_mode()};
  Saved s;
  carve_saved(g, saved, s);
  const int E = g.E, F = g.F;
  const long M = g.M, Ms = g.Ms;
  const float* st = s.st;
  const float* dx2 = g_x_out;
  if (g_y && w->g3) {
    float* t = ws.floats(M * E);
    if (!dry && c.ok()) {
      if (!t) c.rc = HOISDF_ERR_WORKSPACE;
      else if (g.ni == g.nq) c.rc = hoisdf_add_layernorm_bwd(g_y, x_out, nullptr, w->g3, st + 4 * M, st + 5 * M, g_x_out, t, nullptr, G->dg3, G->dbe3, M, E, 0.f, 0, stream);
      else c.rc = hoisdf_layernorm_rows_bwd(g_y, x_out, w->g3, st + 4 * M, st + 5 * M, g_x_out, t, G->dg3, G->dbe3, g.B, g.nq, g.ni, E, stream);
    }
    dx2 = t;
  }
  float* dx1 = ws.floats(M * E); float* df = ws.floats(M * E); float* dh = ws.floats(M * F);
  float* dxq = g.full ? dx : ws.floats(M * E);
  float* da = ws.floats(M * E); float* dO = ws.floats(M * E);
  float* delta = ws.floats((long)g.B * g.H * g.nq);
  if (!dry && (!dx1 || !df || !dh || !dxq || !da || !dO || !delta)) { set_error("encoder_layer_bwd: workspace too small"); return HOISDF_ERR_WORKSPACE; }
  if (!dry && !dx2) { set_error("encoder_layer_bwd: no upstream gradient (g_x_out and g_y both null)"); return HOISDF_ERR_INVALID; }
  enum { MAG_DF = 0, MAG_DH = 1, MAG_DA = 2, MAG_BROWS = 3 };
  const long bmag_bytes = ((long)MAG_BROWS * M + Ms + (long)g.H * g.B) * 4;
  uint32_t* bmag = static_cast<uint32_t*>(ws.take(bmag_bytes));
  const bool mags = layer_mags(c, g) && (dry || bmag);
  auto mg = [&](int i) -> uint32_t* { return mags && bmag ? bmag + (long)i * M : nullptr; };
  uint32_t* const mag_dqkv = mags && bmag ? bmag + (long)MAG_BROWS * M : nullptr;
  uint32_t* const head_do = mags && bmag ? bmag + (long)MAG_BROWS * M + Ms : nullptr;
  auto fm = [&](int i) -> const uint32_t* { return mags && fwd_mags && s.mag ? s.mag + (long)i * M : nullptr; };
  uint32_t* const smag = mags && fwd_mags ? s.mag : nullptr;
  if (mags && !dry && c.ok() && hipMemsetAsync(bmag, 0, (size_t)bmag_bytes, c.st) != hipSuccess) c.rc = HOISDF_ERR_LAUNCH;
  if (!dry && c.ok()) c.rc = add_layernorm_bwd_mag(dx2, s.x1, s.f, w->g2, st + 2 * M, st + 3 * M, nullptr, dx1, df, G->dg2, G->dbe2, M, E, g.p, d->seed[3], nullptr, mg(MAG_DF), stream);
  lin_bwd_input(c, df, E, nullptr, 0.f, w->w2, F, w->img_t_2, dh, F, M, E, F, 0, mg(MAG_DF), mg(MAG_DH));
  lin_bwd_weight(c, df, E, nullptr, 0.f, s.h, F, G->dw2, G->db2, M, E, F, 0, mg(MAG_DF), fm(MAG_H));
  lin_bwd_input(c, dh, F, s.bits, g.p, w->w1, E, w->img_t_1, dx1, E, M, F, E, 1, mg(MAG_DH), nullptr);
  lin_bwd_weight(c, dh, F, s.bits, g.p, s.x1, E, G->dw1, G->db1, M, F, E, 0, mg(MAG_DH), fm(MAG_X1));
  const float* xq2 = g.full ? x : s.xq;
  if (!dry && c.ok()) c.rc = add_layernorm_bwd_mag(dx1, xq2, s.a, w->g1, st, st + M, nullptr, dxq, da, G->dg1, G->dbe1, M, E, g.p, d->seed[1], nullptr, mg(MAG_DA), stream);
  lin_bwd_input(c, da, E, nullptr, 0.f, w->w_out, E, w->img_t_out, dO, E, M, E, E, 0, mg(MAG_DA), nullptr, g.att_h2 ? head_do : nullptr, g.nq);
  lin_bwd_weight(c, da, E, nullptr, 0.f, s.o, E, G->dw_out, G->db_out, M, E, E, 0, mg(MAG_DA), g.att == 2 ? fm(MAG_O) : nullptr);
  const bool amag = mags && g.att_bwd_emu && g.full;
  auto attn_bwd = [&](const float* q, int ldq, const float* k, const float* v, int ldkv, float* dq, float* dk, float* dv) {
    if (g.att_bwd_emu) {
      const long ab = hoisdf_attention_bwd_emu_workspace(g.B, g.H, g.nq, g.S, s.planes ? 1 : 0);
      void* aw = ws.take(ab);
      if (dry || !c.ok()) return;
      if (!aw) { c.rc = HOISDF_ERR_WORKSPACE; return; }
      const bool hm = g.att_h2 && smag && head_do;
      if (g.att_h2 && !hm) { set_error("encoder_layer_bwd: the forward ran the f16x2 attention but the head magnitudes are not available"); c.rc = HOISDF_ERR_INVALID; return; }
      c.rc = attention_bwd_emu_mag(q, ldq, k, ldkv, v, ldkv, s.o, E, dO, E, s.lse, delta, dq, dk, dv, g.B, g.H, g.nq, g.S, g.S, g.p, d->seed[0],
                                   s.planes, aw, ab, amag ? mag_dqkv : nullptr, stream, hm ? head_q(g, smag) : nullptr,
                                   hm ? head_k(g, smag) : nullptr, hm ? head_v(g, smag) : nullptr, hm ? head_do : nullptr);
    } else if (!dry && c.ok()) {
      c.rc = hoisdf_attention_bwd(q, ldq, k, ldkv, v, ldkv, s.o, E, dO, E, s.lse, delta, dq, dk, dv, g.B, g.H, g.nq, g.S, g.S, g.p, d->seed[0], stream);
    }
  };
  if (g.full) {
    float* dqkv = ws.floats(Ms * 3 * E);
    if (!dry && !dqkv) { set_error("encoder_layer_bwd: workspace too small"); return HOISDF_ERR_WORKSPACE; }
    if (g.fused_qkv) attn_bwd(nullptr, 3 * E, nullptr, nullptr, 3 * E, dqkv, dqkv + E, dqkv + 2 * E);
    else attn_bwd(s.qkv, 3 * E, s.qkv + E, s.qkv + 2 * E, 3 * E, dqkv, dqkv + E, dqkv + 2 * E);
    lin_bwd_input(c, dqkv, 3 * E, nullptr, 0.f, w->w_in, E, w->img_t_in, dxq, E, Ms, 3 * E, E, 1, amag ? mag_dqkv : nullptr, nullptr);
    lin_bwd_weight(c, dqkv, 3 * E, nullptr, 0.f, x, E, G->dw_in, G->db_in, Ms, 3 * E, E, 0, amag ? mag_dqkv : nullptr, amag ? d->x_mag : nullptr);
  } else {
    float* dq = ws.floats(M * E); float* dkv = ws.floats(Ms * 2 * E);
    if (!dry && (!dq || !dkv)) { set_error("encoder_layer_bwd: workspace too small"); return HOISDF_ERR_WORKSPACE; }
    if (g.fused_qkv) attn_bwd(nullptr, E, nullptr, nullptr, 2 * E, dq, dkv, dkv + E);
    else attn_bwd(s.qbuf, E, s.kvbuf, s.kvbuf + E, 2 * E, dq, dkv, dkv + E);
    lin_bwd_input(c, dq, E, nullptr, 0.f, w->w_in, E, w->img_t_in_q, dxq, E, M, E, E, 1);
    lin_bwd_weight(c, dq, E, nullptr, 0.f, s.xq, E, G->dw_in, G->db_in, M, E, E);
    lin_bwd_input(c, dkv, 2 * E, nullptr, 0.f, w->w_in + (size_t)E * E, E, w->img_t_in_kv, dx, E, Ms, 2 * E, E, 0);
    lin_bwd_weight(c, dkv, 2 * E, nullptr, 0.f, x, E, G->dw_in + (size_t)E * E, G->db_in ? G->db_in + E : nullptr, Ms, 2 * E, E);
    if (!dry && c.ok()) c.rc = rows_copy_add(dx, (long)g.S * E, dxq, (long)g.nq * E, g.B, g.nq, E, 1, c.st);
  }
  if (c.ok() && !dry && ws.overflow) { set_error("encoder_layer_bwd: workspace too small"); return HOISDF_ERR_WORKSPACE; }
  return c.rc;
}

}
}

using namespace hoisdf;

extern "C" long hoisdf_encoder_layer_saved_bytes(const hoisdf_encoder_layer_desc* d) {
  Geo g;
  if (geometry(d, g) != HOISDF_OK) return -1;
  Bump b(nullptr, 0); Saved s;
  carve_saved(g, b, s);
  return b.off + 256;
// ... 283 lines not shown
```

hoisdf_amd/csrc/pointwise.hip:

```cpp
#include <stdlib.h>

#include "common.h"

namespace hoisdf {

__global__ __launch_bounds__(256) void posenc_kernel(const float* __restrict__ pts, long n_rows,
                                                     float* __restrict__ x0, int ldx0, int col0,
                                                     float* __restrict__ pe, uint32_t* __restrict__ x0_mag) {
  long idx = (long)blockIdx.x * 256 + threadIdx.x;
  const long total = n_rows * 36;
  for (; idx < total; idx += (long)gridDim.x * 256) {
    const long r = idx / 36;
    const int s = (int)(idx - r * 36);
    float val = 0.f;
    if (s < 30) {
      const int k = s / 6, w = s - k * 6, d = w % 3;
      const float f = (float)(1 << k);
      const float arg = pts[r * 3 + d] * f;
      val = (w < 3) ? sinf(arg) : cosf(arg);
      if (pe) pe[r * 30 + s] = val;
    } else if (s < 33) {
      val = pts[r * 3 + (s - 30)];
    }
    if (x0 && col0 + s < ldx0) x0[(size_t)r * ldx0 + col0 + s] = val;
// ... 16 lines not shown
  for (int c = lane; c < ldw; c += 64) W[(size_t)r * ldw + c] = c < in ? vr[c] * sc : 0.f;
  if (norms && lane == 0) norms[r] = nrm;
}

__global__ __launch_bounds__(256) void weightnorm_bwd_kernel(const float* __restrict__ v,
                                                             const float* __restrict__ g,
                                                             const float* __restrict__ dW, int ldw,
                                                             float* __restrict__ dv, float* __restrict__ dg,
                                                             int out, int in) {
  const int lane = threadIdx.x & 63;
  const int r = blockIdx.x * 4 + (threadIdx.x >> 6);
  if (r >= out) return;
  const float* vr = v + (size_t)r * in;
  const float* dr = dW + (size_t)r * ldw;
  float s = 0.f, d = 0.f;
  for (int c = lane; c < in; c += 64) { s += vr[c] * vr[c]; d += dr[c] * vr[c]; }
  s = wave_sum(s); d = wave_sum(d);
  const float nrm = sqrtf(s);
  const float gn = g[r] / nrm;
  const float coef = d / s;
  for (int c = lane; c < in; c += 64) dv[(size_t)r * in + c] = gn * (dr[c] - vr[c] * coef);
  if (lane == 0) dg[r] = d / nrm;
}

__global__ __launch_bounds__(256) void sdf_head_fwd_kernel(const float* __restrict__ h, int ldh,
                                                           const float* __restrict__ w,
                                                           const float* __restrict__ b,
                                                           float* __restrict__ sdf_raw, float* __restrict__ sdf,
                                                           long n_rows, int K, float clampv) {
  const int lane = threadIdx.x & 63;
  long r = (long)blockIdx.x * 4 + (threadIdx.x >> 6);
  for (; r < n_rows; r += (long)gridDim.x * 4) {
    const float* hr = h + (size_t)r * ldh;
    float s = 0.f;
    for (int c = lane * 4; c < K; c += 256) {
      const float4 a = *reinterpret_cast<const float4*>(hr + c);
      const float4 ww = *reinterpret_cast<const float4*>(w + c);
      s += a.x * ww.x + a.y * ww.y + a.z * ww.z + a.w * ww.w;
    }
    s = wave_sum(s);
    if (lane == 0) {
      const float t = tanhf(s + b[0]);
      if (sdf_raw) sdf_raw[r] = t;
      if (sdf) sdf[r] = fminf(fmaxf(t, -clampv), clampv);
    }
  }
}

__global__ __launch_bounds__(256) void sdf_head_bwd_kernel(const float* __restrict__ dsdf,
                                                           const float* __restrict__ sdf_raw,
                                                           const float* __restrict__ h, int ldh,
                                                           const float* __restrict__ w, float* __restrict__ dh,
                                                           int lddh, float* __restrict__ dw, float* __restrict__ db,
                                                           long n_rows, int K, float clampv, DetScratch ds, uint32_t* __restrict__ dh_mag) {
  __shared__ float red[4][512 + 4];
  const int lane = threadIdx.x & 63, wave = threadIdx.x >> 6;
  float4 dwa[2] = {make_float4(0, 0, 0, 0), make_float4(0, 0, 0, 0)};
  float dba = 0.f;
  const long stride = (long)gridDim.x * 4;
  for (long r0 = (long)blockIdx.x * 4 + wave; r0 < n_rows; r0 += 2 * stride) {
    const long r1 = r0 + stride;
    const bool two = r1 < n_rows;
    const float t0 = sdf_raw[r0], t1 = two ? sdf_raw[r1] : 0.f;
    const float g0 = (t0 >= -clampv && t0 <= clampv) ? dsdf[r0] * (1.f - t0 * t0) : 0.f;
    const float g1 = (two && t1 >= -clampv && t1 <= clampv) ? dsdf[r1] * (1.f - t1 * t1) : 0.f;
    const float* h0 = h + (size_t)r0 * ldh;
    const float* h1 = h + (size_t)(two ? r1 : r0) * ldh;
    uint32_t hmax0 = 0u, hmax1 = 0u;
#pragma unroll
    for (int i = 0; i < 2; ++i) {
      const int c = lane * 4 + i * 256;
      if (c < K) {
        const float4 a0 = *reinterpret_cast<const float4*>(h0 + c);
        const float4 a1 = *reinterpret_cast<const float4*>(h1 + c);
        const float4 ww = *reinterpret_cast<const float4*>(w + c);
        const float4 d0 = make_float4(g0 * ww.x, g0 * ww.y, g0 * ww.z, g0 * ww.w), d1 = make_float4(g1 * ww.x, g1 * ww.y, g1 * ww.z, g1 * ww.w);
        *reinterpret_cast<float4*>(dh + (size_t)r0 * lddh + c) = d0;
        if (two) *reinterpret_cast<float4*>(dh + (size_t)r1 * lddh + c) = d1;
        hmax0 = max(hmax0, mag_bits4(d0)); hmax1 = max(hmax1, mag_bits4(d1));
        dwa[i].x += g0 * a0.x + g1 * a1.x; dwa[i].y += g0 * a0.y + g1 * a1.y;
        dwa[i].z += g0 * a0.z + g1 * a1.z; dwa[i].w += g0 * a0.w + g1 * a1.w;
      }
    }
    dba += g0 + g1;
    rowmag_publish_wave(dh_mag, r0, hmax0);
    if (two) rowmag_publish_wave(dh_mag, r1, hmax1);
  }
#pragma unroll
  for (int i = 0; i < 2; ++i) *reinterpret_cast<float4*>(&red[wave][lane * 4 + i * 256]) = dwa[i];
  if (lane == 0) red[wave][512] = dba;
  __syncthreads();
  for (int c = threadIdx.x; c < K; c += 256) red[0][c] = red[0][c] + red[1][c] + red[2][c] + red[3][c];
  if (threadIdx.x == 0) red[1][0] = red[0][512] + red[1][512] + red[2][512] + red[3][512];
  __syncthreads();
  if (threadIdx.x == 0) red[0][K] = red[1][0];
  __syncthreads();
  __shared__ unsigned s_last;
  block_column_sum(dw, K, db, 1, red[0], &s_last, ds);
}

__global__ __launch_bounds__(256) void token_build_fwd_kernel(const float* __restrict__ cam,
                                                              const float* __restrict__ center,
                                                              const float* __restrict__ pe,
                                                              const float* __restrict__ feat, int ldfeat,
                                                              const float* __restrict__ sdf,
                                                              const float* __restrict__ beta_ptr,
                                                              float* __restrict__ tok, int B, int P, int S, int row0,
                                                              int D) {
  const int lane = threadIdx.x & 63;
  const float beta = fmaxf(beta_ptr[0], 2e-3f);
  long r = (long)blockIdx.x * 4 + (threadIdx.x >> 6);
  const long n = (long)B * P;
  for (; r < n; r += (long)gridDim.x * 4) {
    const int b = (int)(r / P), p = (int)(r - (long)b * P);
    const float sig = (1.f / (1.f + expf(-sdf[r] / beta))) / beta;
    float* o = tok + ((size_t)b * S + row0 + p) * D;
    for (int c = lane; c < D; c += 64) {
      float v;
      if (c < 3) v = cam[r * 3 + c] - center[b * 3 + c];
      else if (c < 33) v = pe[r * 30 + (c - 3)];
      else v = feat[(size_t)r * ldfeat + (c - 33)] * sig;
      o[c] = v;
    }
  }
}

__global__ __launch_bounds__(256) void token_build_bwd_kernel(const float* __restrict__ dtok,
                                                              const float* __restrict__ feat, int ldfeat,
                                                              const float* __restrict__ sdf,
                                                              const float* __restrict__ beta_ptr,
                                                              float* __restrict__ dfeat, int lddfeat,
// ... 469 lines not shown
}

extern "C" int hoisdf_posenc_fwd(const float* points, long n_rows, float* x0, int ldx0, int col0, float* pe,
                                 void* stream) {
  return posenc_fwd_mag(points, n_rows, x0, ldx0, col0, pe, nullptr, stream);
}
int hoisdf::posenc_fwd_mag(const float* points, long n_rows, float* x0, int ldx0, int col0, float* pe, uint32_t* x0_mag, void* stream) {
  HOISDF_REQUIRE(points && (x0 || pe) && n_rows >= 0, HOISDF_ERR_INVALID, "posenc_fwd: bad arguments");
  HOISDF_REQUIRE(!x0 || (col0 >= 0 && col0 + 33 <= ldx0), HOISDF_ERR_INVALID,
                 "posenc_fwd: col0=%d + 33 exceeds ldx0=%d", col0, ldx0);
  if (n_rows == 0) return HOISDF_OK;
  long total = n_rows * 36;
  long blocks = (total + 255) / 256;
  if (blocks > 4096) blocks = 4096;
  hipLaunchKernelGGL(posenc_kernel, dim3((unsigned)blocks), dim3(256), 0, as_stream(stream), points, n_rows, x0,
                     ldx0, col0, pe, x0_mag);
  return check_launch("posenc");
}

extern "C" int hoisdf_weightnorm_fwd(const float* v, const float* g, float* W, int ldw, float* norms, int out,
                                     int in, void* stream) {
  HOISDF_REQUIRE(v && g && W && out > 0 && in > 0 && ldw >= in, HOISDF_ERR_INVALID, "weightnorm_fwd: bad arguments");
  hipLaunchKernelGGL(weightnorm_fwd_kernel, dim3(cdiv(out, 4)), dim3(256), 0, as_stream(stream), v, g, W, ldw,
                     norms, out, in);
  return check_launch("weightnorm_fwd");
}

extern "C" int hoisdf_weightnorm_bwd(const float* v, const float* g, const float* dW, int ldw, float* dv,
                                     float* dg, int out, int in, void* stream) {
  HOISDF_REQUIRE(v && g && dW && dv && dg && out > 0 && in > 0 && ldw >= in, HOISDF_ERR_INVALID,
                 "weightnorm_bwd: bad arguments");
  hipLaunchKernelGGL(weightnorm_bwd_kernel, dim3(cdiv(out, 4)), dim3(256), 0, as_stream(stream), v, g, dW, ldw,
                     dv, dg, out, in);
  return check_launch("weightnorm_bwd");
}

extern "C" int hoisdf_sdf_head_fwd(const float* h, int ldh, const float* w, const float* b, float* sdf_raw,
                                   float* sdf, long n_rows, int K, float clamp, void* stream) {
  HOISDF_REQUIRE(h && w && b && (sdf_raw || sdf) && n_rows >= 0, HOISDF_ERR_INVALID, "sdf_head_fwd: null pointer");
  HOISDF_REQUIRE(K > 0 && (K & 3) == 0 && (ldh & 3) == 0 && ldh >= K && ((uintptr_t)h & 15) == 0 &&
                     ((uintptr_t)w & 15) == 0, HOISDF_ERR_INVALID, "sdf_head_fwd: K/ldh must be multiples of 4, 16-byte aligned");
  if (n_rows == 0) return HOISDF_OK;
  hipLaunchKernelGGL(sdf_head_fwd_kernel, dim3(row_grid(n_rows)), dim3(256), 0, as_stream(stream), h, ldh, w, b,
                     sdf_raw, sdf, n_rows, K, clamp);
  return check_launch("sdf_head_fwd");
}

extern "C" int hoisdf_sdf_head_bwd(const float* dsdf, const float* sdf_raw, const float* h, int ldh,
                                   const float* w, float* dh, int lddh, float* dw, float* db, long n_rows, int K,
                                   float clamp, void* stream) {
  return sdf_head_bwd_mag(dsdf, sdf_raw, h, ldh, w, dh, lddh, dw, db, n_rows, K, clamp, nullptr, stream);
}
int hoisdf::sdf_head_bwd_mag(const float* dsdf, const float* sdf_raw, const float* h, int ldh, const float* w, float* dh, int lddh, float* dw,
                             float* db, long n_rows, int K, float clamp, uint32_t* dh_mag, void* stream) {
  HOISDF_REQUIRE(dsdf && sdf_raw && h && w && dh && dw && db && n_rows >= 0, HOISDF_ERR_INVALID,
                 "sdf_head_bwd: null pointer");
  HOISDF_REQUIRE(K > 0 && K <= 512 && (K & 3) == 0 && (ldh & 3) == 0 && (lddh & 3) == 0 && ldh >= K && lddh >= K,
                 HOISDF_ERR_INVALID, "sdf_head_bwd: K must be a multiple of 4 and <= 512");
  if (n_rows == 0) return HOISDF_OK;
  int blocks = row_grid(n_rows);
  if (blocks > 1024) blocks = 1024;
  hipLaunchKernelGGL(sdf_head_bwd_kernel, dim3(blocks), dim3(256), 0, as_stream(stream), dsdf, sdf_raw, h, ldh, w,
                     dh, lddh, dw, db, n_rows, K, clamp, det_scratch((size_t)blocks * (K + 1)), dh_mag);
  return check_launch("sdf_head_bwd");
}

extern "C" int hoisdf_token_build_fwd(const float* cam, const float* center, const float* pe, const float* feat,
                                      int ldfeat, const float* sdf, const float* beta_ptr, float* tok, int B, int P,
                                      int S, int row0, int D, void* stream) {
  HOISDF_REQUIRE(cam && center && pe && feat && sdf && beta_ptr && tok, HOISDF_ERR_INVALID,
                 "token_build_fwd: null pointer");
  HOISDF_REQUIRE(B > 0 && P >= 0 && row0 >= 0 && row0 + P <= S && D > 33 && ldfeat >= D - 33, HOISDF_ERR_INVALID,
                 "token_build_fwd: bad sizes B=%d P=%d S=%d row0=%d D=%d", B, P, S, row0, D);
  if (P == 0) return HOISDF_OK;
  hipLaunchKernelGGL(token_build_fwd_kernel, dim3(row_grid((long)B * P)), dim3(256), 0, as_stream(stream), cam,
                     center, pe, feat, ldfeat, sdf, beta_ptr, tok, B, P, S, row0, D);
  return check_launch("token_build_fwd");
}

extern "C" int hoisdf_token_build_bwd(const float* dtok, const float* feat, int ldfeat, const float* sdf,
                                      const float* beta_ptr, float* dfeat, int lddfeat, float* dbeta, int B, int P,
                                      int S, int row0, int D, void* stream) {
  HOISDF_REQUIRE(dtok && feat && sdf && beta_ptr && dfeat, HOISDF_ERR_INVALID, "token_build_bwd: null pointer");
  HOISDF_REQUIRE(B > 0 && P >= 0 && row0 >= 0 && row0 + P <= S && D > 33 && ldfeat >= D - 33 && lddfeat >= D - 33,
                 HOISDF_ERR_INVALID, "token_build_bwd: bad sizes");
  if (P == 0) return HOISDF_OK;
  int blocks = row_grid((long)B * P);
  if (blocks > 1024) blocks = 1024;
  hipLaunchKernelGGL(token_build_bwd_kernel, dim3(blocks), dim3(256), 0, as_stream(stream), dtok, feat, ldfeat,
                     sdf, beta_ptr, dfeat, lddfeat, dbeta, B, P, S, row0, D, det_scratch((size_t)blocks), (float*)nullptr);
  return check_launch("token_build_bwd");
}

extern "C" int hoisdf_token_build_bwd_partials(void) { return 1024; }

extern "C" int hoisdf_token_build_bwd_ordered(const float* dtok, const float* feat, int ldfeat, const float* sdf,
                                              const float* beta_ptr, float* dfeat, int lddfeat, float* dbeta, float* partials,
                                              int B, int P, int S, int row0, int D, void* stream) {
  HOISDF_REQUIRE(dtok && feat && sdf && beta_ptr && dfeat && dbeta && partials, HOISDF_ERR_INVALID, "token_build_bwd_ordered: null pointer");
  HOISDF_REQUIRE(B > 0 && P >= 0 && row0 >= 0 && row0 + P <= S && D > 33 && ldfeat >= D - 33 && lddfeat >= D - 33,
                 HOISDF_ERR_INVALID, "token_build_bwd_ordered: bad sizes");
  if (P == 0) return HOISDF_OK;
  int blocks = row_grid((long)B * P);
  if (blocks > 1024) blocks = 1024;
  DetScratch off{};
  hipLaunchKernelGGL(token_build_bwd_kernel, dim3(blocks), dim3(256), 0, as_stream(stream), dtok, feat, ldfeat,
                     sdf, beta_ptr, dfeat, lddfeat, dbeta, B, P, S, row0, D, off, partials);
  hipLaunchKernelGGL(token_beta_finish_kernel, dim3(1), dim3(64), 0, as_stream(stream), partials, blocks, dbeta);
  return check_launch("token_build_bwd_ordered");
}

extern "C" int hoisdf_add_layernorm_fwd(const float* x, const float* r, const float* gamma, const float* beta,
                                        float* y, float* mean, float* rstd, long M, int D, float eps, float drop_p,
                                        uint64_t seed, void* stream) {
  return add_layernorm_fwd_mag(x, r, gamma, beta, y, mean, rstd, M, D, eps, drop_p, seed, nullptr, stream);
}
// ... 105 lines not shown
```

hoisdf_amd/csrc/runtime.hip:

```cpp
#include <string.h>
#include <stdarg.h>
#include <stdio.h>
#include <stdlib.h>

#include "common.h"

namespace hoisdf {

static thread_local char g_err[512] = "";

void set_error(const char* fmt, ...) {
  va_list ap;
  va_start(ap, fmt);
  vsnprintf(g_err, sizeof(g_err), fmt, ap);
  va_end(ap);
}

int check_launch(const char* what) {
  hipError_t e = hipGetLastError();
  if (e != hipSuccess) {
    set_error("%s: %s", what, hipGetErrorString(e));
    return HOISDF_ERR_LAUNCH;
  }
  return HOISDF_OK;
}

static int g_det = -1;
static int g_gemm_emu = 1;

bool gemm_emu_mode() {
  static int env = -1;
  if (env < 0) {
    const char* e = getenv("HOISDF_GEMM");
    env = (e && strcmp(e, "f32") == 0) ? 0 : 1;
    if (!env) g_gemm_emu = 0;
  }
  return g_gemm_emu != 0;
}

bool deterministic_mode() {
  if (g_det < 0) {
    const char* e = getenv("HOISDF_DETERMINISTIC");
    g_det = (e && e[0] && e[0] != '0') ? 1 : 0;
  }
  return g_det == 1;
}

DetScratch det_scratch(size_t floats) {
  static float* part = nullptr;
  static unsigned* ticket = nullptr;
  static size_t cap = 0;
  DetScratch d{nullptr, nullptr, 0};
  if (!deterministic_mode()) return d;
  if (floats > cap || !ticket) {
    if (part) (void)hipFree(part);
    cap = floats < (1u << 20) ? (1u << 20) : floats;
    if (hipMalloc(&part, cap * sizeof(float)) != hipSuccess) { part = nullptr; cap = 0; return d; }
    if (!ticket) {
      if (hipMalloc(&ticket, sizeof(unsigned)) != hipSuccess) { ticket = nullptr; return d; }
      (void)hipMemset(ticket, 0, sizeof(unsigned));
    }
  }
  d.part = part; d.ticket = ticket; d.on = 1;
  return d;
}

}

extern "C" void hoisdf_set_gemm_emu(int on) { (void)hoisdf::gemm_emu_mode(); hoisdf::g_gemm_emu = on ? 1 : 0; }
extern "C" int hoisdf_get_gemm_emu(void) { return hoisdf::gemm_emu_mode() ? 1 : 0; }
extern "C" void hoisdf_set_deterministic(int on) { hoisdf::g_det = on ? 1 : 0; }
extern "C" int hoisdf_get_deterministic(void) { return hoisdf::deterministic_mode() ? 1 : 0; }
extern "C" const char* hoisdf_version(void) { return "hoisdf-hip 0.1 (gfx950)"; }
extern "C" const char* hoisdf_last_error(void) { return hoisdf::g_err; }
```

hoisdf_amd/csrc/sdf_query.hip:

```cpp
#include "common.h"

using namespace hoisdf;

namespace {
constexpr int HID0 = 512, LAT = 256, PF = 33, H1 = 223, X0 = LAT + PF, CAT_K = 516, X0_COL = 224;
constexpr int CAT_LD = 544;
inline long align64(long v) { return (v + 63) / 64 * 64; }
constexpr long EMU_MIN_ROWS_Q = 2048;

inline long emu_scratch_bytes(int C) {
  const long a = hoisdf_linear_emu_image_bytes(HID0, C), b = hoisdf_linear_emu_image_bytes(HID0, CAT_K);
  return ((a > b ? a : b) + 255) / 256 * 256;
}

int layer(const float* x, int ldx, const float* W, int ldw, const float* b, float* y, int ldy, long M, int N, int K,
          int K_pad, float drop_p, uint64_t seed, void* emu_img, const void* given, void* stream, const uint32_t* x_mag = nullptr,
          uint32_t* y_mag = nullptr, bool* y_has = nullptr) {
  if (y_has) *y_has = false;
  if (emu_img && M >= EMU_MIN_ROWS_Q && hoisdf_linear_emu_supported(x, ldx, K_pad) && (K_pad + 15) / 16 == (K + 15) / 16) {
    if (!given) { if (int rc = hoisdf_linear_emu_prepare(W, ldw, N, K, 0, emu_img, stream)) return rc; }
    if (y_has) *y_has = y_mag != nullptr;
    return linear_fwd_emu_mag(x, ldx, given ? given : emu_img, b, y, ldy, M, N, K_pad, 1, drop_p, seed, nullptr, x_mag, y_mag, stream);
  }
  return hoisdf_linear_fwd(x, ldx, W, ldw, b, y, ldy, M, N, K, 1, drop_p, seed, nullptr, stream);
// ... 188 lines not shown
}

extern "C" long hoisdf_sdf_query_train_saved_bytes(long n_rows, int C) {
  if (n_rows <= 0 || C <= 0) return 0;
  Bump b(nullptr, 0); TrainSaved s;
  train_carve(n_rows, C, b, s);
  return b.off + 256;
}

static int sdf_train_forward(const hoisdf_pyramid* pyr, const float* points, const int32_t* sample_idx, long n, int rps, const float* center,
                             const float* cam_intr, float scale, int img_h, int img_w, const hoisdf_sdf_weights* w, float clamp, float drop_p,
                             uint64_t seed, float* sdf, float* pe, float* cam_out, Bump& saved, Bump& ws, bool dry, void* stream) {
  Ctx c{as_stream(stream), stream, &ws, dry, gemm_emu_mode()};
  TrainSaved s;
  const int C = w ? w->C : 1;
  train_carve(n, C, saved, s);
  const bool mags = train_mags(c, n) && !dry && s.mag;
  if (!dry) saved_mags().put(s.mag, mags);
  auto mg = [&](int i) -> uint32_t* { return mags ? s.mag + (long)i * n : nullptr; };
  if (!dry) {
    if (mags) c.rc = hipMemsetAsync(s.mag, 0, (size_t)TM_N * n * 4, c.st) == hipSuccess ? HOISDF_OK : HOISDF_ERR_LAUNCH;
    if (c.ok()) c.rc = project_gather_fwd_mag(pyr, points, sample_idx, n, rps, center, cam_intr, scale, img_h, img_w, s.feat, C, cam_out, nullptr, mg(TM_FEAT), stream);
    if (c.ok()) c.rc = hipMemsetAsync(s.cat, 0, sizeof(float) * n * CAT_LD, c.st) == hipSuccess ? HOISDF_OK : HOISDF_ERR_LAUNCH;
  }
  float* x0 = dry ? nullptr : s.cat + X0_COL;
  lin_fwd(c, s.feat, C, w->sdfin_w0, C, w->emu_img[0], w->sdfin_b0, s.ha, HID0, n, HID0, C, 1, 0.f, 0, s.ba, 0, mg(TM_FEAT), mg(TM_HA));
  lin_fwd(c, s.ha, HID0, w->sdfin_w1, HID0, w->emu_img[1], w->sdfin_b1, x0, CAT_LD, n, LAT, HID0, 1, 0.f, 0, s.bf, 0, mg(TM_HA), mg(TM_CAT));
  if (!dry && c.ok()) c.rc = posenc_fwd_mag(points, n, s.cat, CAT_LD, X0_COL + LAT, pe, mg(TM_CAT), stream);
  lin_fwd(c, x0, CAT_LD, w->dec_w0, w->dec_ld0, w->emu_img[2], w->dec_b0, s.h0, HID0, n, HID0, X0, 1, drop_p, seed, s.b0, X0 + 3, mg(TM_CAT), mg(TM_H0));
  lin_fwd(c, s.h0, HID0, w->dec_w1, HID0, w->emu_img[3], w->dec_b1, s.cat, CAT_LD, n, H1 + 1, HID0, 1, drop_p, seed + 1, s.b1, 0, mg(TM_H0), mg(TM_CAT));
  lin_fwd(c, s.cat, CAT_LD, w->dec_w2, CAT_K, w->emu_img[4], w->dec_b2, s.h2, HID0, n, HID0, CAT_K, 1, drop_p, seed + 2, s.b2, 0, mg(TM_CAT), mg(TM_H2));
  lin_fwd(c, s.h2, HID0, w->dec_w3, HID0, w->emu_img[5], w->dec_b3, s.h3, HID0, n, HID0, HID0, 1, drop_p, seed + 3, s.b3, 0, mg(TM_H2), nullptr);
  if (!dry && c.ok()) c.rc = hoisdf_sdf_head_fwd(s.h3, HID0, w->dec_w4, w->dec_b4, s.raw, sdf, n, HID0, clamp, stream);
  return c.rc;
}

static int sdf_train_backward(const hoisdf_pyramid_grad* dpyr, const float* points, const int32_t* sample_idx, long n, int rps, const float* center,
                              const float* cam_intr, float scale, int img_h, int img_w, const hoisdf_sdf_weights* w, float clamp, float drop_p,
                              const float* d_sdf, const hoisdf_sdf_weight_grads* G, Bump& saved, Bump& ws, bool dry, void* stream) {
  Ctx c{as_stream(stream), stream, &ws, dry, gemm_emu_mode()};
  TrainSaved s;
  const int C = w ? w->C : 1;
  train_carve(n, C, saved, s);
  float* dh3 = ws.floats(n * HID0); float* dh2 = ws.floats(n * HID0); float* dcat = ws.floats(n * CAT_LD); float* dh0 = ws.floats(n * HID0);
  float* dha = ws.floats(n * HID0); float* dfeat = ws.floats(n * (long)C);
  if (!dry && (!dh3 || !dh2 || !dcat || !dh0 || !dha || !dfeat)) { set_error("sdf_query_bwd: workspace too small"); return HOISDF_ERR_WORKSPACE; }
  enum { BM_DH3 = 0, BM_DH2 = 1, BM_DCAT = 2, BM_DH0 = 3, BM_DHA = 4, BM_N = 5 };
  uint32_t* bmag = static_cast<uint32_t*>(ws.take((long)BM_N * n * 4));
  const bool mags = train_mags(c, n) && !dry && bmag && s.mag;
  const bool fmags = mags && saved_mags().get(s.mag) != 0;
  auto mg = [&](int i) -> uint32_t* { return mags ? bmag + (long)i * n : nullptr; };
  auto fm = [&](int i) -> const uint32_t* { return fmags ? s.mag + (long)i * n : nullptr; };
  if (mags) c.rc = hipMemsetAsync(bmag, 0, (size_t)BM_N * n * 4, c.st) == hipSuccess ? HOISDF_OK : HOISDF_ERR_LAUNCH;
  if (!dry && c.ok()) c.rc = sdf_head_bwd_mag(d_sdf, s.raw, s.h3, HID0, w->dec_w4, dh3, HID0, G->d_dec_w4, G->d_dec_b4, n, HID0, clamp, mg(BM_DH3), stream);
  lin_bwd_input(c, dh3, HID0, s.b3, drop_p, w->dec_w3, HID0, w->emu_img_t[5], dh2, HID0, n, HID0, HID0, 0, mg(BM_DH3), mg(BM_DH2));
  lin_bwd_weight(c, dh3, HID0, s.b3, drop_p, s.h2, HID0, G->d_dec_w3, G->d_dec_b3, n, HID0, HID0, 0, mg(BM_DH3), fm(TM_H2));
  lin_bwd_input(c, dh2, HID0, s.b2, drop_p, w->dec_w2, CAT_K, w->emu_img_t[4], dcat, CAT_LD, n, HID0, CAT_K, 0, mg(BM_DH2), mg(BM_DCAT));
  lin_bwd_weight(c, dh2, HID0, s.b2, drop_p, s.cat, CAT_LD, G->d_dec_w2, G->d_dec_b2, n, HID0, CAT_K, 0, mg(BM_DH2), fm(TM_CAT));
  lin_bwd_input(c, dcat, CAT_LD, s.b1, drop_p, w->dec_w1, HID0, w->emu_img_t[3], dh0, HID0, n, H1 + 1, HID0, 0, mg(BM_DCAT), mg(BM_DH0));
  lin_bwd_weight(c, dcat, CAT_LD, s.b1, drop_p, s.h0, HID0, G->d_dec_w1, G->d_dec_b1, n, H1 + 1, HID0, 0, mg(BM_DCAT), fm(TM_H0));
  float* dx0 = dry ? nullptr : dcat + X0_COL;
  const float* x0 = dry ? nullptr : s.cat + X0_COL;
  lin_bwd_input(c, dh0, HID0, s.b0, drop_p, w->dec_w0, w->dec_ld0, w->emu_img_t[2], dx0, CAT_LD, n, HID0, X0, 1, mg(BM_DH0), nullptr);
  lin_bwd_weight(c, dh0, HID0, s.b0, drop_p, x0, CAT_LD, G->d_dec_w0, G->d_dec_b0, n, HID0, X0, X0 + 3, mg(BM_DH0), fm(TM_CAT));
  lin_bwd_input(c, dx0, CAT_LD, s.bf, 0.f, w->sdfin_w1, HID0, w->emu_img_t[1], dha, HID0, n, LAT, HID0, 0, nullptr, mg(BM_DHA));
  lin_bwd_weight(c, dx0, CAT_LD, s.bf, 0.f, s.ha, HID0, G->d_sdfin_w1, G->d_sdfin_b1, n, LAT, HID0, 0, nullptr, fm(TM_HA));
  lin_bwd_input(c, dha, HID0, s.ba, 0.f, w->sdfin_w0, C, w->emu_img_t[0], dfeat, C, n, HID0, C, 0, mg(BM_DHA), nullptr);
  lin_bwd_weight(c, dha, HID0, s.ba, 0.f, s.feat, C, G->d_sdfin_w0, G->d_sdfin_b0, n, HID0, C, 0, mg(BM_DHA), fm(TM_FEAT));
  if (!dry && c.ok() && dpyr)
    c.rc = hoisdf_project_gather_bwd(dpyr, points, sample_idx, n, rps, center, cam_intr, scale, img_h, img_w, dfeat, C, stream);
  if (c.ok() && !dry && ws.overflow) { set_error("sdf_query_bwd: workspace too small"); return HOISDF_ERR_WORKSPACE; }
  return c.rc;
}

extern "C" long hoisdf_sdf_query_train_workspace_bytes(long n_rows, int C, int backward_pass) {
  if (n_rows <= 0 || C <= 0) return 0;
  hoisdf_sdf_weights w{}; w.C = C; w.dec_ld0 = X0;
  hoisdf_sdf_weight_grads G{};
  Bump saved(nullptr, 0), ws(nullptr, 0);
  if (backward_pass) (void)sdf_train_backward(nullptr, nullptr, nullptr, n_rows, 1, nullptr, nullptr, 1.f, 1, 1, &w, 0.f, 0.f, nullptr, &G, saved, ws, true, nullptr);
  else (void)sdf_train_forward(nullptr, nullptr, nullptr, n_rows, 1, nullptr, nullptr, 1.f, 1, 1, &w, 0.f, 0.f, 0, nullptr, nullptr, nullptr, saved, ws, true, nullptr);
  return ws.off + 256;
}

extern "C" int hoisdf_sdf_query_train_fwd(const hoisdf_pyramid* pyr, const float* points, const int32_t* sample_idx, long n_rows, int rows_per_sample,
                                          const float* center, const float* cam_intr, float scale, int img_h, int img_w,
                                          const hoisdf_sdf_weights* w, float clamp, float drop_p, uint64_t seed, float* sdf, float* pe,
                                          float* cam_out, void* saved, long saved_bytes, void* workspace, long workspace_bytes, void* stream) {
  HOISDF_REQUIRE(pyr && points && w && sdf && saved && workspace && center && cam_intr, HOISDF_ERR_INVALID, "sdf_query_train_fwd: null pointer");
  HOISDF_REQUIRE(n_rows > 0 && n_rows < (1L << 31) && w->C > 0 && w->C % 4 == 0 && w->dec_ld0 >= X0, HOISDF_ERR_INVALID, "sdf_query_train_fwd: bad sizes");
  HOISDF_REQUIRE(drop_p >= 0.f && drop_p < 1.f, HOISDF_ERR_INVALID, "sdf_query_train_fwd: drop_p=%f", drop_p);
  HOISDF_REQUIRE(saved_bytes >= hoisdf_sdf_query_train_saved_bytes(n_rows, w->C), HOISDF_ERR_WORKSPACE, "sdf_query_train_fwd: saved buffer of %ld bytes, need %ld",
                 saved_bytes, hoisdf_sdf_query_train_saved_bytes(n_rows, w->C));
  Bump sv(saved, saved_bytes), ws(workspace, workspace_bytes);
  int rc = sdf_train_forward(pyr, points, sample_idx, n_rows, rows_per_sample, center, cam_intr, scale, img_h, img_w, w, clamp, drop_p, seed, sdf, pe, cam_out,
                             sv, ws, false, stream);
  if (rc == HOISDF_OK && (sv.overflow || ws.overflow)) rc = HOISDF_ERR_WORKSPACE;
  if (rc == HOISDF_ERR_WORKSPACE) set_error("sdf_query_train_fwd: workspace (%ld bytes) too small", workspace_bytes);
  return rc;
}

extern "C" int hoisdf_sdf_query_bwd(const hoisdf_pyramid_grad* dpyr, const float* points, const int32_t* sample_idx, long n_rows, int rows_per_sample,
                                    const float* center, const float* cam_intr, float scale, int img_h, int img_w, const hoisdf_sdf_weights* w,
                                    float clamp, float drop_p, const void* saved, long saved_bytes, const float* d_sdf,
                                    const hoisdf_sdf_weight_grads* grads, void* workspace, long workspace_bytes, void* stream) {
  HOISDF_REQUIRE(points && w && saved && d_sdf && grads && workspace && center && cam_intr, HOISDF_ERR_INVALID, "sdf_query_bwd: null pointer");
  HOISDF_REQUIRE(grads->d_sdfin_w0 && grads->d_sdfin_b0 && grads->d_sdfin_w1 && grads->d_sdfin_b1 && grads->d_dec_w0 && grads->d_dec_b0 && grads->d_dec_w1 &&
                     grads->d_dec_b1 && grads->d_dec_w2 && grads->d_dec_b2 && grads->d_dec_w3 && grads->d_dec_b3 && grads->d_dec_w4 && grads->d_dec_b4,
                 HOISDF_ERR_INVALID, "sdf_query_bwd: every weight gradient buffer is required (zero-filled)");
  HOISDF_REQUIRE(n_rows > 0 && n_rows < (1L << 31) && saved_bytes >= hoisdf_sdf_query_train_saved_bytes(n_rows, w->C), HOISDF_ERR_INVALID,
                 "sdf_query_bwd: bad sizes / saved buffer");
  Bump sv(const_cast<void*>(saved), saved_bytes), ws(workspace, workspace_bytes);
  int rc = sdf_train_backward(dpyr, points, sample_idx, n_rows, rows_per_sample, center, cam_intr, scale, img_h, img_w, w, clamp, drop_p, d_sdf, grads, sv, ws,
                              false, stream);
  if (rc == HOISDF_ERR_WORKSPACE) set_error("sdf_query_bwd: workspace (%ld bytes) too small", workspace_bytes);
  return rc;
}
```

include/hoisdf.h:

```cpp
#ifndef HOISDF_H_
#define HOISDF_H_

#include <stdint.h>

#ifdef __cplusplus
extern "C" {
#endif

#define HOISDF_VERSION_MAJOR 0
#define HOISDF_VERSION_MINOR 1

typedef enum hoisdf_status {
  HOISDF_OK = 0,
  HOISDF_ERR_INVALID = -1,
  HOISDF_ERR_LAUNCH = -2,
  HOISDF_ERR_TOO_FEW = -3,
  HOISDF_ERR_WORKSPACE = -4
} hoisdf_status;

#define HOISDF_MAX_LEVELS 8

typedef struct hoisdf_pyramid {
  int n_levels;
  int B;
  const float* data[HOISDF_MAX_LEVELS];
  int C[HOISDF_MAX_LEVELS];
  int H[HOISDF_MAX_LEVELS];
  int W[HOISDF_MAX_LEVELS];
} hoisdf_pyramid;

typedef struct hoisdf_pyramid_grad {
  int n_levels;
  int B;
  float* data[HOISDF_MAX_LEVELS];
  int C[HOISDF_MAX_LEVELS];
  int H[HOISDF_MAX_LEVELS];
  int W[HOISDF_MAX_LEVELS];
} hoisdf_pyramid_grad;

const char* hoisdf_version(void);
const char* hoisdf_last_error(void);
void hoisdf_set_deterministic(int on);
void hoisdf_set_gemm_emu(int on);
int hoisdf_get_gemm_emu(void);
int hoisdf_get_deterministic(void);

int hoisdf_project_gather_fwd(const hoisdf_pyramid* pyr, const float* points,
                              const int32_t* sample_idx, long n_rows, int rows_per_sample,
                              const float* center, const float* cam_intr, float scale,
                              int img_h, int img_w, float* feat, int ldf, float* cam_out,
                              float* uv_out, void* stream);
int hoisdf_project_gather_bwd(const hoisdf_pyramid_grad* dpyr, const float* points,
                              const int32_t* sample_idx, long n_rows, int rows_per_sample,
                              const float* center, const float* cam_intr, float scale,
                              int img_h, int img_w, const float* dfeat, int ldf, void* stream);

int hoisdf_linear_fwd(const float* x, int ldx, const float* W, int ldw, const float* bias,
                      float* y, int ldy, long M, int N, int K, int act, float drop_p,
                      uint64_t seed, uint32_t* relu_bits, void* stream);
int hoisdf_linear_bwd_input(const float* dy, int lddy, const uint32_t* relu_bits, float drop_p,
                            const float* W, int ldw, float* dx, int lddx, long M, int N, int K,
                            int accumulate ,
                            void* stream);
long hoisdf_linear_bwd_weight_workspace(long M, int N, int K);
int hoisdf_linear_bwd_weight(const float* dy, int lddy, const uint32_t* relu_bits, float drop_p,
                             const float* x, int ldx, float* dW, int lddw, float* db, long M, int N,
                             int K, float* workspace, long workspace_floats, void* stream);
long hoisdf_linear_emu_image_bytes(int rows, int K);
int hoisdf_linear_emu_prepare(const float* W, int ldw, int N, int K, int transpose, void* image, void* stream);
typedef struct hoisdf_emu_prep_item {
  const float* W;
  void* image;
  long first_block;
  int ldw, N, K, transpose;
} hoisdf_emu_prep_item;
long hoisdf_linear_emu_prepare_blocks(int N, int K, int transpose);
int hoisdf_linear_emu_prepare_batch(const hoisdf_emu_prep_item* d_items, int n, long total_blocks, void* stream);
int hoisdf_linear_emu_supported(const float* a, long lda, int contraction);
int hoisdf_linear_emu_pieces(void);
long hoisdf_mag_words(long rows);
int hoisdf_mag_measure(const float* x, long ldx, long M, int K, uint32_t* words, void* stream);
long hoisdf_head_mag_words(long M, int groups, int L);
int hoisdf_head_mag_measure(const float* x, long ldx, long M, int groups, int L, uint32_t* words, void* stream);
int hoisdf_linear_fwd_emu_heads(const float* x, int ldx, const void* w_image, const float* bias, float* y, int ldy, long M, int N,
                                int K, const uint32_t* x_mag, uint32_t* y_mag, uint32_t* y_heads, int L, void* stream);
int hoisdf_linear_bwd_input_emu_heads(const float* dy, int lddy, const void* wt_image, float* dx, int lddx, long M, int N, int K,
                                      const uint32_t* dy_mag, uint32_t* dx_mag, uint32_t* dx_heads, int L, void* stream);
int hoisdf_linear_fwd_emu_mag(const float* x, int ldx, const void* w_image, const float* bias, float* y, int ldy, long M, int N,
                              int K, int act, float drop_p, uint64_t seed, uint32_t* relu_bits, const uint32_t* x_mag,
                              uint32_t* y_mag, void* stream);
int hoisdf_linear_bwd_input_emu_mag(const float* dy, int lddy, const uint32_t* relu_bits, float drop_p, const void* wt_image,
                                    float* dx, int lddx, long M, int N, int K, int accumulate, const uint32_t* dy_mag,
                                    uint32_t* dx_mag, void* stream);
int hoisdf_linear_bwd_weight_emu_mag(const float* dy, int lddy, const uint32_t* relu_bits, float drop_p, const float* x, int ldx,
                                     float* dW, int lddw, float* db, long M, int N, int K, float* workspace, long workspace_floats,
                                     const uint32_t* dy_mag, const uint32_t* x_mag, void* stream);
int hoisdf_linear_fwd_emu(const float* x, int ldx, const void* w_image, const float* bias, float* y, int ldy, long M, int N,
                          int K, int act, float drop_p, uint64_t seed, uint32_t* relu_bits, void* stream);
// ... 417 lines not shown
```

Before: 448.2.

## Apply ReLU/dropout gradient mask at producer store instead of consumer operand load

Adds an output bitmap mask to the emulated bwd-input GEMM epilogue and the SDF head backward so the next layer's ReLU/dropout mask is applied when dx is stored. Downstream bwd-input and bwd-weight GEMMs then read the gradient as already masked and skip per-element bit lookups in their operand loads, keeping only the dropout scale via a new ascale_on flag. The change threads this through the SDF query backward chain and the heads MLP, and it is on by default behind a runtime toggle. In exchange, the epilogue gains extra bitmap reads and branches, and correctness depends on the premasked flags chaining consistently between layers.

```diff
diff --git a/hoisdf_amd/_lib.py b/hoisdf_amd/_lib.py
--- a/hoisdf_amd/_lib.py
+++ b/hoisdf_amd/_lib.py
@@ -233,6 +233,7 @@
 }
 _RET = {"hoisdf_version": C.c_char_p, "hoisdf_last_error": C.c_char_p}
 _OTHER = {"hoisdf_set_deterministic": ([_I], None), "hoisdf_set_gemm_emu": ([_I], None), "hoisdf_get_gemm_emu": ([], C.c_int), "hoisdf_get_deterministic": ([], C.c_int),
+          "hoisdf_set_grad_mask_at_store": ([_I], None), "hoisdf_get_grad_mask_at_store": ([], C.c_int),
           "hoisdf_mano_dirs_image_floats": ([], C.c_long),
           "hoisdf_point_loss_blocks": ([_L], C.c_int),
           "hoisdf_bn_workspace_floats": ([_L, _I], C.c_long),
diff --git a/hoisdf_amd/csrc/chain.h b/hoisdf_amd/csrc/chain.h
--- a/hoisdf_amd/csrc/chain.h
+++ b/hoisdf_amd/csrc/chain.h
@@ -75,16 +75,23 @@
   if (emu_small(c, M, x, ldx, W, ldw, N, K)) { c.rc = hoisdf_linear_fwd_emu_small(x, ldx, W, ldw, b, y, ldy, M, N, K, act, p, seed, bits, c.stream); return; }
   c.rc = hoisdf_linear_fwd(x, ldx, W, ldw, b, y, ldy, M, N, K, act, p, seed, bits, c.stream);
 }
+inline bool premask_ok(const StoreMask* m, const uint32_t* stored_mag) {
+  return grad_mask_at_store_mode() && store_mask_ok(m) && (stored_mag != nullptr || !emu_form_h2());
+}
 void lin_bwd_input(Ctx& c, const float* dy, int lddy, const uint32_t* bits, float p, const float* W, int ldw, const void* img_t, float* dx,
                    int lddx, long M, int N, int K, int accumulate, const uint32_t* dy_mag = nullptr, uint32_t* dx_mag = nullptr,
-                   uint32_t* dx_heads = nullptr, int head_L = 0) {
+                   uint32_t* dx_heads = nullptr, int head_L = 0, const StoreMask* out_mask = nullptr, bool* masked = nullptr,
+                   bool dy_premasked = false) {
+  if (masked) *masked = false;
   if (!c.ok()) return;
-  if (!bits) p = 0.f;
+  if (!bits) { p = 0.f; dy_premasked = false; }
   if (emu_rows(c, M, dy, lddy, N)) {
     const void* im = image_of(c, img_t, W, ldw, N, K, 1);
     if (c.dry || !c.ok()) return;
+    const bool mask = premask_ok(out_mask, accumulate ? nullptr : dx_mag);
     c.rc = linear_bwd_input_emu_mag(dy, lddy, bits, p, im, dx, lddx, M, N, K, accumulate, dy_mag, accumulate ? nullptr : dx_mag, c.stream,
-                                    accumulate ? nullptr : dx_heads, head_L);
+                                    accumulate ? nullptr : dx_heads, head_L, dy_premasked ? 1 : 0, mask ? out_mask : nullptr);
+    if (masked) *masked = mask && c.ok();
     return;
   }
   if (c.dry) return;
@@ -92,9 +99,9 @@
   c.rc = hoisdf_linear_bwd_input(dy, lddy, bits, p, W, ldw, dx, lddx, M, N, K, accumulate, c.stream);
 }
 void lin_bwd_weight(Ctx& c, const float* dy, int lddy, const uint32_t* bits, float p, const float* x, int ldx, float* dW, float* db, long M,
-                    int N, int K, int K_pad = 0, const uint32_t* dy_mag = nullptr, const uint32_t* x_mag = nullptr) {
+                    int N, int K, int K_pad = 0, const uint32_t* dy_mag = nullptr, const uint32_t* x_mag = nullptr, bool dy_premasked = false) {
   if (!c.ok()) return;
-  if (!bits) p = 0.f;
+  if (!bits) { p = 0.f; dy_premasked = false; }
   if (K_pad < K) K_pad = K;
   const bool emu = c.emu && M >= EMU_DW_MIN_ROWS && (N < K ? N : K) >= 64 && N % 4 == 0 && K_pad % 4 == 0 && lddy % 4 == 0 && ldx % 4 == 0 &&
                    (c.dry || (al16(dy) && al16(x) && al16(dW)));
@@ -103,7 +110,8 @@
     float* w = c.ws->floats(nws > 4 ? nws : 4);
     if (!c.dry) {
       if (!w) { c.rc = HOISDF_ERR_WORKSPACE; return; }
-      if (dy_mag || x_mag) c.rc = linear_bwd_weight_emu_mag(dy, lddy, bits, p, x, ldx, dW, K_pad, db, M, N, K_pad, w, nws, dy_mag, x_mag, c.stream);
+      if (dy_mag || x_mag || (dy_premasked && !emu_form_h2()))
+        c.rc = linear_bwd_weight_emu_mag(dy, lddy, bits, p, x, ldx, dW, K_pad, db, M, N, K_pad, w, nws, dy_mag, x_mag, c.stream, dy_premasked ? 1 : 0);
       else c.rc = hoisdf_linear_bwd_weight_emu(dy, lddy, bits, p, x, ldx, dW, K_pad, db, M, N, K_pad, w, nws, c.stream);
     }
     return;
diff --git a/hoisdf_amd/csrc/common.h b/hoisdf_amd/csrc/common.h
--- a/hoisdf_amd/csrc/common.h
+++ b/hoisdf_amd/csrc/common.h
@@ -109,18 +109,20 @@
 int linear_fwd_emu_mag(const float* x, int ldx, const void* w_image, const float* bias, float* y, int ldy, long M, int N, int K, int act,
                        float drop_p, uint64_t seed, uint32_t* relu_bits, const uint32_t* x_mag, uint32_t* y_mag, void* stream,
                        uint32_t* y_heads = nullptr, int head_L = 0);
+struct StoreMask { const uint32_t* bits; int ldbits, col0, cols; };
+inline bool store_mask_ok(const StoreMask* m) { return m && m->bits && m->col0 >= 0 && m->cols > 0 && m->col0 % 4 == 0 && m->cols % 4 == 0 && m->cols <= 32 * m->ldbits; }
 int linear_bwd_input_emu_mag(const float* dy, int lddy, const uint32_t* relu_bits, float drop_p, const void* wt_image, float* dx, int lddx,
                              long M, int N, int K, int accumulate, const uint32_t* dy_mag, uint32_t* dx_mag, void* stream,
-                             uint32_t* dx_heads = nullptr, int head_L = 0);
+                             uint32_t* dx_heads = nullptr, int head_L = 0, int dy_premasked = 0, const StoreMask* out_mask = nullptr);
 int linear_bwd_weight_emu_mag(const float* dy, int lddy, const uint32_t* relu_bits, float drop_p, const float* x, int ldx, float* dW, int lddw,
                               float* db, long M, int N, int K, float* workspace, long workspace_floats, const uint32_t* dy_mag,
-                              const uint32_t* x_mag, void* stream);
+                              const uint32_t* x_mag, void* stream, int dy_premasked = 0);
 int project_gather_fwd_mag(const hoisdf_pyramid* pyr, const float* points, const int32_t* sample_idx, long n_rows, int rows_per_sample,
                            const float* center, const float* cam_intr, float scale, int img_h, int img_w, float* feat, int ldf, float* cam_out,
                            float* uv_out, uint32_t* feat_mag, void* stream);
 int posenc_fwd_mag(const float* points, long n_rows, float* x0, int ldx0, int col0, float* pe, uint32_t* x0_mag, void* stream);
 int sdf_head_bwd_mag(const float* dsdf, const float* sdf_raw, const float* h, int ldh, const float* w, float* dh, int lddh, float* dw,
-                     float* db, long n_rows, int K, float clamp, uint32_t* dh_mag, void* stream);
+                     float* db, long n_rows, int K, float clamp, uint32_t* dh_mag, void* stream, const StoreMask* dh_mask = nullptr);
 int add_layernorm_fwd_mag(const float* x, const float* r, const float* gamma, const float* beta, float* y, float* mean, float* rstd, long M,
                           int D, float eps, float drop_p, uint64_t seed, uint32_t* y_mag, void* stream);
 int add_layernorm_bwd_mag(const float* dy, const float* x, const float* r, const float* gamma, const float* mean, const float* rstd,
@@ -144,6 +146,7 @@
 int maxpool_launch(const float* x, int ldx, float* y, int ldy, int B, int H, int W, int C, hipStream_t st);
 
 bool deterministic_mode();
+bool grad_mask_at_store_mode();
 bool gemm_emu_mode();
 struct DetScratch {
   float* part;
diff --git a/hoisdf_amd/csrc/gemm_emu.h b/hoisdf_amd/csrc/gemm_emu.h
--- a/hoisdf_amd/csrc/gemm_emu.h
+++ b/hoisdf_amd/csrc/gemm_emu.h
@@ -43,6 +43,8 @@
   float* C; int ldc;
   const float* bias;
   const uint32_t* abits; int ldbits; float ascale;
+  int ascale_on;
+  const uint32_t* obits; int ldobits, ocol0, ocols;
   uint32_t* bits_out; int ldbits_out;
   int M, N, K;
   int act; float drop_p, inv_keep; uint32_t thresh; uint64_t seed;
@@ -57,6 +59,7 @@
   const float* dy; long lddy;
   const float* x; long ldx;
   const uint32_t* bits; int ldbits; float ascale;
+  int ascale_on;
   float* C; long c_split_stride;
   float* colsum; long colsum_split_stride;
   int M, N, K;
@@ -250,6 +253,17 @@
     float* w = reinterpret_cast<float*>(lds) + wave * (32 * ES);
 #pragma unroll
     for (int i = 0; i < 4; ++i) {
+      uint32_t ow[32 / RPI];
+#pragma unroll
+      for (int p = 0; p < 32 / RPI; ++p) ow[p] = 0xfu;
+      if (g.obits) {
+        const int mc = n0 + wn * WN_ + (lane % LPR) * 4 - g.ocol0;
+        if (mc >= 0 && mc < g.ocols) {
+          const uint32_t* bp = g.obits + (size_t)(m0 + wm * 128 + i * 32 + lane / LPR) * g.ldobits + (mc >> 5);
+#pragma unroll
+          for (int p = 0; p < 32 / RPI; ++p) ow[p] = bp[(size_t)p * RPI * g.ldobits] >> (mc & 31);
+        }
+      }
 #pragma unroll
       for (int j = 0; j < NJ_; ++j)
 #pragma unroll
@@ -275,6 +289,10 @@
           const float4 old = *cp;
           v.x += old.x; v.y += old.y; v.z += old.z; v.w += old.w;
         }
+        if (g.obits) {
+          v.x = (ow[p] & 1u) ? v.x : 0.f; v.y = (ow[p] & 2u) ? v.y : 0.f;
+          v.z = (ow[p] & 4u) ? v.z : 0.f; v.w = (ow[p] & 8u) ? v.w : 0.f;
+        }
         typedef float v4f_ __attribute__((ext_vector_type(4)));
 #ifdef H2_ABL_NOSTORE
         if (g.seed != 0x5eed5eed5eedull) continue;
@@ -293,7 +311,12 @@
           const int row = rbase + i * 32 + (r & 3) + 8 * (r >> 2), col = cbase + j * 32;
           if (row < g.M && col < g.N) {
             float* cp = g.C + (size_t)row * g.ldc + col;
-            *cp = g.beta ? *cp + acc[i][j][r] : acc[i][j][r];
+            float v = g.beta ? *cp + acc[i][j][r] : acc[i][j][r];
+            if (g.obits) {
+              const int mc = col - g.ocol0;
+              if (mc >= 0 && mc < g.ocols && !((g.obits[(size_t)row * g.ldobits + (mc >> 5)] >> (mc & 31)) & 1u)) v = 0.f;
+            }
+            *cp = v;
           }
         }
     if (g.amax_out) {
diff --git a/hoisdf_amd/csrc/gemm_emu.hip b/hoisdf_amd/csrc/gemm_emu.hip
--- a/hoisdf_amd/csrc/gemm_emu.hip
+++ b/hoisdf_amd/csrc/gemm_emu.hip
@@ -244,8 +244,10 @@
 
 int hoisdf::linear_bwd_input_emu_mag(const float* dy, int lddy, const uint32_t* relu_bits, float drop_p, const void* wt_image, float* dx,
                                      int lddx, long M, int N, int K, int accumulate, const uint32_t* dy_mag, uint32_t* dx_mag,
-                                     void* stream, uint32_t* dx_heads, int head_L) {
+                                     void* stream, uint32_t* dx_heads, int head_L, int dy_premasked, const StoreMask* out_mask) {
   HOISDF_REQUIRE(M == 0 || (dy && wt_image && dx), HOISDF_ERR_INVALID, "linear_bwd_input_emu: null pointer");
+  HOISDF_REQUIRE(!out_mask || (store_mask_ok(out_mask) && out_mask->col0 + out_mask->cols <= K), HOISDF_ERR_INVALID,
+                 "linear_bwd_input_emu: output bitmap (columns and first column multiples of 4, inside dx and the bitmap's row)");
   HOISDF_REQUIRE(M >= 0 && N > 0 && K > 0 && lddy >= N && lddx >= K && M < (1L << 31) && drop_p >= 0.f && drop_p < 1.f,
                  HOISDF_ERR_INVALID, "linear_bwd_input_emu: bad sizes");
   if (M == 0) return HOISDF_OK;
@@ -253,7 +255,9 @@
                  "linear_bwd_input_emu: dy must be 16-byte aligned with lddy and N multiples of 4");
   EmuArgs g{};
   g.A = dy; g.lda = lddy; g.Bimg = static_cast<const u32x4*>(wt_image);
-  g.abits = relu_bits; g.ldbits = (N + 31) / 32; g.ascale = 1.f / (1.f - drop_p);
+  g.abits = dy_premasked ? nullptr : relu_bits; g.ldbits = (N + 31) / 32; g.ascale = 1.f / (1.f - drop_p);
+  g.ascale_on = relu_bits != nullptr;
+  if (out_mask) { g.obits = out_mask->bits; g.ldobits = out_mask->ldbits; g.ocol0 = out_mask->col0; g.ocols = out_mask->cols; }
   g.C = dx; g.ldc = lddx; g.M = (int)M; g.N = K; g.K = N;
   g.inv_keep = 1.f;
   g.beta = accumulate ? 1 : 0;
@@ -276,7 +280,7 @@
 namespace {
 int bwd_weight_emu(const float* dy, int lddy, const uint32_t* relu_bits, float drop_p, const float* x, int ldx, float* dW, int lddw,
                    float* db, long M, int N, int K, float* workspace, long workspace_floats, bool h2, const uint32_t* dy_mag,
-                   const uint32_t* x_mag, void* stream) {
+                   const uint32_t* x_mag, void* stream, int dy_premasked = 0) {
   HOISDF_REQUIRE(dW && (M == 0 || (dy && x)), HOISDF_ERR_INVALID, "linear_bwd_weight_emu: null pointer");
   HOISDF_REQUIRE(M > 0 && N > 0 && K > 0 && lddy >= N && ldx >= K && lddw == K && M < (1L << 31) && drop_p >= 0.f && drop_p < 1.f,
                  HOISDF_ERR_INVALID, "linear_bwd_weight_emu: bad sizes (a dense dW, lddw == K, is required)");
@@ -285,9 +289,10 @@
   hipStream_t st = as_stream(stream);
   DwArgs g{};
   g.dy = dy; g.lddy = lddy; g.x = x; g.ldx = ldx;
-  g.bits = relu_bits; g.ldbits = (N + 31) / 32; g.ascale = 1.f / (1.f - drop_p);
+  const int dtk = dw_tile(K);
+  g.bits = (dy_premasked && dtk == 256) ? nullptr : relu_bits; g.ldbits = (N + 31) / 32; g.ascale = 1.f / (1.f - drop_p);
+  g.ascale_on = relu_bits != nullptr;
   g.M = (int)M; g.N = N; g.K = K;
-  const int dtk = dw_tile(K);
   g.tiles_n = cdiv(N, DT); g.tiles_k = cdiv(K, dtk);
   plan_dw(M, N, K, g.splitk, g.m_per_split);
   const long need = g.splitk > 1 ? (long)g.splitk * ((long)N * K + N) : 0;
@@ -327,8 +332,8 @@
 }
 int hoisdf::linear_bwd_weight_emu_mag(const float* dy, int lddy, const uint32_t* relu_bits, float drop_p, const float* x, int ldx,
                                       float* dW, int lddw, float* db, long M, int N, int K, float* workspace, long workspace_floats,
-                                      const uint32_t* dy_mag, const uint32_t* x_mag, void* stream) {
-  return bwd_weight_emu(dy, lddy, relu_bits, drop_p, x, ldx, dW, lddw, db, M, N, K, workspace, workspace_floats, form_h2(), dy_mag, x_mag, stream);
+                                      const uint32_t* dy_mag, const uint32_t* x_mag, void* stream, int dy_premasked) {
+  return bwd_weight_emu(dy, lddy, relu_bits, drop_p, x, ldx, dW, lddw, db, M, N, K, workspace, workspace_floats, form_h2(), dy_mag, x_mag, stream, dy_premasked);
 }
 extern "C" int hoisdf_linear_bwd_weight_emu_mag(const float* dy, int lddy, const uint32_t* relu_bits, float drop_p, const float* x,
                                                 int ldx, float* dW, int lddw, float* db, long M, int N, int K, float* workspace,
diff --git a/hoisdf_amd/csrc/gemm_emu_b3.hip b/hoisdf_amd/csrc/gemm_emu_b3.hip
--- a/hoisdf_amd/csrc/gemm_emu_b3.hip
+++ b/hoisdf_amd/csrc/gemm_emu_b3.hip
@@ -160,7 +160,7 @@
 #undef PHASE
 #undef STAGE_ALL
 #undef LOAD_ALL
-  emu_epilogue<TM, TN, NJ>(g, acc, st0, m0, n0, wm, wn, wave, lane, l31, kh, MASK ? g.ascale : 1.f);
+  emu_epilogue<TM, TN, NJ>(g, acc, st0, m0, n0, wm, wn, wave, lane, l31, kh, g.ascale_on ? g.ascale : 1.f);
 }
 
 int emu_b3_prepare(const float* W, int ldw, int R, int Kc, int transpose, void* image, hipStream_t st) {
diff --git a/hoisdf_amd/csrc/gemm_emu_dw.hip b/hoisdf_amd/csrc/gemm_emu_dw.hip
--- a/hoisdf_amd/csrc/gemm_emu_dw.hip
+++ b/hoisdf_amd/csrc/gemm_emu_dw.hip
@@ -351,10 +351,10 @@
 #undef MM
 #undef DPHASE
 #undef DSTAGE_ALL
-  const float post = MASK ? g.ascale : 1.f;
+  const float post = g.ascale_on ? g.ascale : 1.f;
   u32x4* lds = s0;
   DW2_STORE_COLSUM();
-  DW_EPILOGUE(DT, MASK ? acc[i][j][r] * post : acc[i][j][r]);
+  DW_EPILOGUE(DT, acc[i][j][r] * post);
 }
 
 template <bool MASK, bool HASDB>
@@ -458,10 +458,10 @@
 #undef DHPHASE
 #undef DSTAGE_ALL
   const float unscale = h2_inv_scale(am_dy) * h2_inv_scale(am_x);
-  const float post = MASK ? g.ascale : 1.f;
+  const float post = g.ascale_on ? g.ascale : 1.f;
   u32x4* lds = lds_all;
   DW2_STORE_COLSUM();
-  DW_EPILOGUE(DT, acc[i][j][r] * (MASK ? post * unscale : unscale));
+  DW_EPILOGUE(DT, acc[i][j][r] * (post * unscale));
 }
 
 __global__ __launch_bounds__(1024) void emu_reduce_partials_kernel(const float* __restrict__ part, long stride, int splits,
diff --git a/hoisdf_amd/csrc/gemm_emu_h2.hip b/hoisdf_amd/csrc/gemm_emu_h2.hip
--- a/hoisdf_amd/csrc/gemm_emu_h2.hip
+++ b/hoisdf_amd/csrc/gemm_emu_h2.hip
@@ -165,7 +165,7 @@
   for (int i = 0; i < 4; ++i) sAr[i] = h2_scale(wrow[i]);
   HSTAGE_ALL(st0, 0);
   HLOAD_ALL(1);
-  rpost[tid] = h2_inv_scale(wpost) * g.b_scale[1] * (MASK ? g.ascale : 1.f);
+  rpost[tid] = h2_inv_scale(wpost) * g.b_scale[1] * (g.ascale_on ? g.ascale : 1.f);
   __syncthreads();
 #pragma unroll
   for (int i = 0; i < 4; ++i) { aL[i] = HLA(st0, 1, i); aH[i] = HLA(st0, 0, i); }
diff --git a/hoisdf_amd/csrc/heads.hip b/hoisdf_amd/csrc/heads.hip
--- a/hoisdf_amd/csrc/heads.hip
+++ b/hoisdf_amd/csrc/heads.hip
@@ -57,6 +57,7 @@
   uint32_t* mg = chain_mags(c, M, m->n_layers + 1);
   const bool fwd_mags = mg && s.mag && saved_mags().get(s.mag) != 0;
   const uint32_t* g_mag = nullptr;
+  bool g_masked = false;
   if (mg && emu_rows(c, M, dy, lddy, m->dims[last + 1])) {
     if ((c.rc = emu_mag_measure(dy, lddy, M, m->dims[last + 1], mg + (long)(last + 1) * M, c.st)) != HOISDF_OK) return;
     g_mag = mg + (long)(last + 1) * M;
@@ -66,15 +67,17 @@
     const int ldin = i > 0 ? m->dims[i] : ldx;
     const uint32_t* in_mag = !fwd_mags ? nullptr : i > 0 ? (emu_rows(c, M, i > 1 ? s.h[i - 2] : x, i > 1 ? m->dims[i - 1] : ldx, m->dims[i - 1]) ? s.mag + (long)i * M : nullptr)
                                                          : (x_mag ? x_mag : (emu_rows(c, M, x, ldx, m->dims[0]) ? s.mag : nullptr));
-    lin_bwd_weight(c, g, ldg, s.bits[i], 0.f, in, ldin, G->dw[i], G->db[i], M, m->dims[i + 1], m->dims[i], 0, g_mag, g_mag ? in_mag : nullptr);
+    lin_bwd_weight(c, g, ldg, s.bits[i], 0.f, in, ldin, G->dw[i], G->db[i], M, m->dims[i + 1], m->dims[i], 0, g_mag, g_mag ? in_mag : nullptr, g_masked);
     if (i == 0 && !dx) break;
     float* gin = i > 0 ? c.ws->floats(M * m->dims[i]) : dx;
     const int ldgin = i > 0 ? m->dims[i] : lddx;
     if (!c.dry && c.ok() && !gin) { c.rc = HOISDF_ERR_WORKSPACE; return; }
     uint32_t* gin_mag = mg && i > 0 && emu_rows(c, M, g, ldg, m->dims[i + 1]) ? mg + (long)i * M : nullptr;
+    const StoreMask gin_mask{i > 0 ? s.bits[i - 1] : nullptr, (int)bits_words(m->dims[i]), 0, m->dims[i]};
+    bool gin_masked = false;
     lin_bwd_input(c, g, ldg, s.bits[i], 0.f, m->w[i], m->dims[i], m->img_t[i], gin, ldgin, M, m->dims[i + 1], m->dims[i], i == 0 ? accumulate_dx : 0,
-                  g_mag, gin_mag);
-    g = gin; ldg = ldgin; g_mag = gin_mag;
+                  g_mag, gin_mag, nullptr, 0, &gin_mask, &gin_masked, g_masked);
+    g = gin; ldg = ldgin; g_mag = gin_mag; g_masked = gin_masked;
   }
 }
 const uint32_t* enc_mag(const Ctx& c, const hoisdf_mlp* m, const float* x, int ldx, long M, const MlpSaved& s) {
diff --git a/hoisdf_amd/csrc/layers.hip b/hoisdf_amd/csrc/layers.hip
--- a/hoisdf_amd/csrc/layers.hip
+++ b/hoisdf_amd/csrc/layers.hip
@@ -214,10 +214,12 @@
   uint32_t* const smag = mags && fwd_mags ? s.mag : nullptr;
   if (mags && !dry && c.ok() && hipMemsetAsync(bmag, 0, (size_t)bmag_bytes, c.st) != hipSuccess) c.rc = HOISDF_ERR_LAUNCH;
   if (!dry && c.ok()) c.rc = add_layernorm_bwd_mag(dx2, s.x1, s.f, w->g2, st + 2 * M, st + 3 * M, nullptr, dx1, df, G->dg2, G->dbe2, M, E, g.p, d->seed[3], nullptr, mg(MAG_DF), stream);
-  lin_bwd_input(c, df, E, nullptr, 0.f, w->w2, F, w->img_t_2, dh, F, M, E, F, 0, mg(MAG_DF), mg(MAG_DH));
+  const StoreMask dh_mask{s.bits, (F + 31) / 32, 0, F};
+  bool dh_masked = false;
+  lin_bwd_input(c, df, E, nullptr, 0.f, w->w2, F, w->img_t_2, dh, F, M, E, F, 0, mg(MAG_DF), mg(MAG_DH), nullptr, 0, &dh_mask, &dh_masked);
   lin_bwd_weight(c, df, E, nullptr, 0.f, s.h, F, G->dw2, G->db2, M, E, F, 0, mg(MAG_DF), fm(MAG_H));
-  lin_bwd_input(c, dh, F, s.bits, g.p, w->w1, E, w->img_t_1, dx1, E, M, F, E, 1, mg(MAG_DH), nullptr);
-  lin_bwd_weight(c, dh, F, s.bits, g.p, s.x1, E, G->dw1, G->db1, M, F, E, 0, mg(MAG_DH), fm(MAG_X1));
+  lin_bwd_input(c, dh, F, s.bits, g.p, w->w1, E, w->img_t_1, dx1, E, M, F, E, 1, mg(MAG_DH), nullptr, nullptr, 0, nullptr, nullptr, dh_masked);
+  lin_bwd_weight(c, dh, F, s.bits, g.p, s.x1, E, G->dw1, G->db1, M, F, E, 0, mg(MAG_DH), fm(MAG_X1), dh_masked);
   const float* xq2 = g.full ? x : s.xq;
   if (!dry && c.ok()) c.rc = add_layernorm_bwd_mag(dx1, xq2, s.a, w->g1, st, st + M, nullptr, dxq, da, G->dg1, G->dbe1, M, E, g.p, d->seed[1], nullptr, mg(MAG_DA), stream);
   lin_bwd_input(c, da, E, nullptr, 0.f, w->w_out, E, w->img_t_out, dO, E, M, E, E, 0, mg(MAG_DA), nullptr, g.att_h2 ? head_do : nullptr, g.nq);
diff --git a/hoisdf_amd/csrc/pointwise.hip b/hoisdf_amd/csrc/pointwise.hip
--- a/hoisdf_amd/csrc/pointwise.hip
+++ b/hoisdf_amd/csrc/pointwise.hip
@@ -92,7 +92,8 @@
                                                            const float* __restrict__ h, int ldh,
                                                            const float* __restrict__ w, float* __restrict__ dh,
                                                            int lddh, float* __restrict__ dw, float* __restrict__ db,
-                                                           long n_rows, int K, float clampv, DetScratch ds, uint32_t* __restrict__ dh_mag) {
+                                                           long n_rows, int K, float clampv, DetScratch ds, uint32_t* __restrict__ dh_mag,
+                                                           const uint32_t* __restrict__ mbits, int ldmbits) {
   __shared__ float red[4][512 + 4];
   const int lane = threadIdx.x & 63, wave = threadIdx.x >> 6;
   float4 dwa[2] = {make_float4(0, 0, 0, 0), make_float4(0, 0, 0, 0)};
@@ -115,8 +116,12 @@
         const float4 a1 = *reinterpret_cast<const float4*>(h1 + c);
         const float4 ww = *reinterpret_cast<const float4*>(w + c);
         const float4 d0 = make_float4(g0 * ww.x, g0 * ww.y, g0 * ww.z, g0 * ww.w), d1 = make_float4(g1 * ww.x, g1 * ww.y, g1 * ww.z, g1 * ww.w);
-        *reinterpret_cast<float4*>(dh + (size_t)r0 * lddh + c) = d0;
-        if (two) *reinterpret_cast<float4*>(dh + (size_t)r1 * lddh + c) = d1;
+        const uint32_t n0 = mbits ? mbits[(size_t)r0 * ldmbits + (c >> 5)] >> (c & 31) : 0xfu;
+        const uint32_t n1 = (mbits && two) ? mbits[(size_t)r1 * ldmbits + (c >> 5)] >> (c & 31) : 0xfu;
+        *reinterpret_cast<float4*>(dh + (size_t)r0 * lddh + c) =
+            make_float4((n0 & 1u) ? d0.x : 0.f, (n0 & 2u) ? d0.y : 0.f, (n0 & 4u) ? d0.z : 0.f, (n0 & 8u) ? d0.w : 0.f);
+        if (two) *reinterpret_cast<float4*>(dh + (size_t)r1 * lddh + c) =
+            make_float4((n1 & 1u) ? d1.x : 0.f, (n1 & 2u) ? d1.y : 0.f, (n1 & 4u) ? d1.z : 0.f, (n1 & 8u) ? d1.w : 0.f);
         hmax0 = max(hmax0, mag_bits4(d0)); hmax1 = max(hmax1, mag_bits4(d1));
         dwa[i].x += g0 * a0.x + g1 * a1.x; dwa[i].y += g0 * a0.y + g1 * a1.y;
         dwa[i].z += g0 * a0.z + g1 * a1.z; dwa[i].w += g0 * a0.w + g1 * a1.w;
@@ -692,16 +697,18 @@
   return sdf_head_bwd_mag(dsdf, sdf_raw, h, ldh, w, dh, lddh, dw, db, n_rows, K, clamp, nullptr, stream);
 }
 int hoisdf::sdf_head_bwd_mag(const float* dsdf, const float* sdf_raw, const float* h, int ldh, const float* w, float* dh, int lddh, float* dw,
-                             float* db, long n_rows, int K, float clamp, uint32_t* dh_mag, void* stream) {
+                             float* db, long n_rows, int K, float clamp, uint32_t* dh_mag, void* stream, const StoreMask* dh_mask) {
   HOISDF_REQUIRE(dsdf && sdf_raw && h && w && dh && dw && db && n_rows >= 0, HOISDF_ERR_INVALID,
                  "sdf_head_bwd: null pointer");
   HOISDF_REQUIRE(K > 0 && K <= 512 && (K & 3) == 0 && (ldh & 3) == 0 && (lddh & 3) == 0 && ldh >= K && lddh >= K,
                  HOISDF_ERR_INVALID, "sdf_head_bwd: K must be a multiple of 4 and <= 512");
+  HOISDF_REQUIRE(!dh_mask || (store_mask_ok(dh_mask) && dh_mask->col0 == 0 && dh_mask->cols == K), HOISDF_ERR_INVALID, "sdf_head_bwd: the bitmap must cover dh's K columns");
   if (n_rows == 0) return HOISDF_OK;
   int blocks = row_grid(n_rows);
   if (blocks > 1024) blocks = 1024;
   hipLaunchKernelGGL(sdf_head_bwd_kernel, dim3(blocks), dim3(256), 0, as_stream(stream), dsdf, sdf_raw, h, ldh, w,
-                     dh, lddh, dw, db, n_rows, K, clamp, det_scratch((size_t)blocks * (K + 1)), dh_mag);
+                     dh, lddh, dw, db, n_rows, K, clamp, det_scratch((size_t)blocks * (K + 1)), dh_mag, dh_mask ? dh_mask->bits : nullptr,
+                     dh_mask ? dh_mask->ldbits : 0);
   return check_launch("sdf_head_bwd");
 }
 
diff --git a/hoisdf_amd/csrc/runtime.hip b/hoisdf_amd/csrc/runtime.hip
--- a/hoisdf_amd/csrc/runtime.hip
+++ b/hoisdf_amd/csrc/runtime.hip
@@ -38,6 +38,10 @@
   return g_gemm_emu != 0;
 }
 
+static int g_mask_at_store = 1;
+
+bool grad_mask_at_store_mode() { return g_mask_at_store != 0; }
+
 bool deterministic_mode() {
   if (g_det < 0) {
     const char* e = getenv("HOISDF_DETERMINISTIC");
@@ -69,6 +73,8 @@
 
 extern "C" void hoisdf_set_gemm_emu(int on) { (void)hoisdf::gemm_emu_mode(); hoisdf::g_gemm_emu = on ? 1 : 0; }
 extern "C" int hoisdf_get_gemm_emu(void) { return hoisdf::gemm_emu_mode() ? 1 : 0; }
+extern "C" void hoisdf_set_grad_mask_at_store(int on) { hoisdf::g_mask_at_store = on ? 1 : 0; }
+extern "C" int hoisdf_get_grad_mask_at_store(void) { return hoisdf::grad_mask_at_store_mode() ? 1 : 0; }
 extern "C" void hoisdf_set_deterministic(int on) { hoisdf::g_det = on ? 1 : 0; }
 extern "C" int hoisdf_get_deterministic(void) { return hoisdf::deterministic_mode() ? 1 : 0; }
 extern "C" const char* hoisdf_version(void) { return "hoisdf-hip 0.1 (gfx950)"; }
diff --git a/hoisdf_amd/csrc/sdf_query.hip b/hoisdf_amd/csrc/sdf_query.hip
--- a/hoisdf_amd/csrc/sdf_query.hip
+++ b/hoisdf_amd/csrc/sdf_query.hip
@@ -264,21 +264,24 @@
   auto mg = [&](int i) -> uint32_t* { return mags ? bmag + (long)i * n : nullptr; };
   auto fm = [&](int i) -> const uint32_t* { return fmags ? s.mag + (long)i * n : nullptr; };
   if (mags) c.rc = hipMemsetAsync(bmag, 0, (size_t)BM_N * n * 4, c.st) == hipSuccess ? HOISDF_OK : HOISDF_ERR_LAUNCH;
-  if (!dry && c.ok()) c.rc = sdf_head_bwd_mag(d_sdf, s.raw, s.h3, HID0, w->dec_w4, dh3, HID0, G->d_dec_w4, G->d_dec_b4, n, HID0, clamp, mg(BM_DH3), stream);
-  lin_bwd_input(c, dh3, HID0, s.b3, drop_p, w->dec_w3, HID0, w->emu_img_t[5], dh2, HID0, n, HID0, HID0, 0, mg(BM_DH3), mg(BM_DH2));
-  lin_bwd_weight(c, dh3, HID0, s.b3, drop_p, s.h2, HID0, G->d_dec_w3, G->d_dec_b3, n, HID0, HID0, 0, mg(BM_DH3), fm(TM_H2));
-  lin_bwd_input(c, dh2, HID0, s.b2, drop_p, w->dec_w2, CAT_K, w->emu_img_t[4], dcat, CAT_LD, n, HID0, CAT_K, 0, mg(BM_DH2), mg(BM_DCAT));
-  lin_bwd_weight(c, dh2, HID0, s.b2, drop_p, s.cat, CAT_LD, G->d_dec_w2, G->d_dec_b2, n, HID0, CAT_K, 0, mg(BM_DH2), fm(TM_CAT));
-  lin_bwd_input(c, dcat, CAT_LD, s.b1, drop_p, w->dec_w1, HID0, w->emu_img_t[3], dh0, HID0, n, H1 + 1, HID0, 0, mg(BM_DCAT), mg(BM_DH0));
-  lin_bwd_weight(c, dcat, CAT_LD, s.b1, drop_p, s.h0, HID0, G->d_dec_w1, G->d_dec_b1, n, H1 + 1, HID0, 0, mg(BM_DCAT), fm(TM_H0));
+  auto sm = [&](const uint32_t* bits, int cols) { return StoreMask{bits, (int)bits_words(cols), 0, cols}; };
+  const StoreMask m3 = sm(s.b3, HID0), m2 = sm(s.b2, HID0), m1 = sm(s.b1, H1 + 1), m0 = sm(s.b0, HID0), mf = sm(s.bf, LAT), ma = sm(s.ba, HID0);
+  bool k3 = !dry && premask_ok(&m3, mg(BM_DH3)), k2 = false, k1 = false, k0 = false, kf = false, ka = false;
+  if (!dry && c.ok()) c.rc = sdf_head_bwd_mag(d_sdf, s.raw, s.h3, HID0, w->dec_w4, dh3, HID0, G->d_dec_w4, G->d_dec_b4, n, HID0, clamp, mg(BM_DH3), stream, k3 ? &m3 : nullptr);
+  lin_bwd_input(c, dh3, HID0, s.b3, drop_p, w->dec_w3, HID0, w->emu_img_t[5], dh2, HID0, n, HID0, HID0, 0, mg(BM_DH3), mg(BM_DH2), nullptr, 0, &m2, &k2, k3);
+  lin_bwd_weight(c, dh3, HID0, s.b3, drop_p, s.h2, HID0, G->d_dec_w3, G->d_dec_b3, n, HID0, HID0, 0, mg(BM_DH3), fm(TM_H2), k3);
+  lin_bwd_input(c, dh2, HID0, s.b2, drop_p, w->dec_w2, CAT_K, w->emu_img_t[4], dcat, CAT_LD, n, HID0, CAT_K, 0, mg(BM_DH2), mg(BM_DCAT), nullptr, 0, &m1, &k1, k2);
+  lin_bwd_weight(c, dh2, HID0, s.b2, drop_p, s.cat, CAT_LD, G->d_dec_w2, G->d_dec_b2, n, HID0, CAT_K, 0, mg(BM_DH2), fm(TM_CAT), k2);
+  lin_bwd_input(c, dcat, CAT_LD, s.b1, drop_p, w->dec_w1, HID0, w->emu_img_t[3], dh0, HID0, n, H1 + 1, HID0, 0, mg(BM_DCAT), mg(BM_DH0), nullptr, 0, &m0, &k0, k1);
+  lin_bwd_weight(c, dcat, CAT_LD, s.b1, drop_p, s.h0, HID0, G->d_dec_w1, G->d_dec_b1, n, H1 + 1, HID0, 0, mg(BM_DCAT), fm(TM_H0), k1);
   float* dx0 = dry ? nullptr : dcat + X0_COL;
   const float* x0 = dry ? nullptr : s.cat + X0_COL;
-  lin_bwd_input(c, dh0, HID0, s.b0, drop_p, w->dec_w0, w->dec_ld0, w->emu_img_t[2], dx0, CAT_LD, n, HID0, X0, 1, mg(BM_DH0), nullptr);
-  lin_bwd_weight(c, dh0, HID0, s.b0, drop_p, x0, CAT_LD, G->d_dec_w0, G->d_dec_b0, n, HID0, X0, X0 + 3, mg(BM_DH0), fm(TM_CAT));
-  lin_bwd_input(c, dx0, CAT_LD, s.bf, 0.f, w->sdfin_w1, HID0, w->emu_img_t[1], dha, HID0, n, LAT, HID0, 0, nullptr, mg(BM_DHA));
-  lin_bwd_weight(c, dx0, CAT_LD, s.bf, 0.f, s.ha, HID0, G->d_sdfin_w1, G->d_sdfin_b1, n, LAT, HID0, 0, nullptr, fm(TM_HA));
-  lin_bwd_input(c, dha, HID0, s.ba, 0.f, w->sdfin_w0, C, w->emu_img_t[0], dfeat, C, n, HID0, C, 0, mg(BM_DHA), nullptr);
-  lin_bwd_weight(c, dha, HID0, s.ba, 0.f, s.feat, C, G->d_sdfin_w0, G->d_sdfin_b0, n, HID0, C, 0, mg(BM_DHA), fm(TM_FEAT));
+  lin_bwd_input(c, dh0, HID0, s.b0, drop_p, w->dec_w0, w->dec_ld0, w->emu_img_t[2], dx0, CAT_LD, n, HID0, X0, 1, mg(BM_DH0), nullptr, nullptr, 0, &mf, &kf, k0);
+  lin_bwd_weight(c, dh0, HID0, s.b0, drop_p, x0, CAT_LD, G->d_dec_w0, G->d_dec_b0, n, HID0, X0, X0 + 3, mg(BM_DH0), fm(TM_CAT), k0);
+  lin_bwd_input(c, dx0, CAT_LD, s.bf, 0.f, w->sdfin_w1, HID0, w->emu_img_t[1], dha, HID0, n, LAT, HID0, 0, nullptr, mg(BM_DHA), nullptr, 0, &ma, &ka, kf);
+  lin_bwd_weight(c, dx0, CAT_LD, s.bf, 0.f, s.ha, HID0, G->d_sdfin_w1, G->d_sdfin_b1, n, LAT, HID0, 0, nullptr, fm(TM_HA), kf);
+  lin_bwd_input(c, dha, HID0, s.ba, 0.f, w->sdfin_w0, C, w->emu_img_t[0], dfeat, C, n, HID0, C, 0, mg(BM_DHA), nullptr, nullptr, 0, nullptr, nullptr, ka);
+  lin_bwd_weight(c, dha, HID0, s.ba, 0.f, s.feat, C, G->d_sdfin_w0, G->d_sdfin_b0, n, HID0, C, 0, mg(BM_DHA), fm(TM_FEAT), ka);
   if (!dry && c.ok() && dpyr)
     c.rc = hoisdf_project_gather_bwd(dpyr, points, sample_idx, n, rps, center, cam_intr, scale, img_h, img_w, dfeat, C, stream);
   if (c.ok() && !dry && ws.overflow) { set_error("sdf_query_bwd: workspace too small"); return HOISDF_ERR_WORKSPACE; }
diff --git a/include/hoisdf.h b/include/hoisdf.h
--- a/include/hoisdf.h
+++ b/include/hoisdf.h
@@ -44,6 +44,8 @@
 void hoisdf_set_gemm_emu(int on);
 int hoisdf_get_gemm_emu(void);
 int hoisdf_get_deterministic(void);
+void hoisdf_set_grad_mask_at_store(int on);
+int hoisdf_get_grad_mask_at_store(void);
 
 int hoisdf_project_gather_fwd(const hoisdf_pyramid* pyr, const float* points,
                               const int32_t* sample_idx, long n_rows, int rows_per_sample,
```

After: 450.8, median of 6. Within noise of the previous version (+0.6%).
